# feifeibear/long-context-attention

Hardware: AMD Instinct MI355X
Metric: attention TFLOP/s (algorithmic, causal fwd+bwd) + iter ms of LongContextAttention at seqlen 64K, ulysses x ring (higher is better)
Workload: dtype bf16

## Files before the change

### include/usp_hip.h

```cpp
#ifndef USP_HIP_H
#define USP_HIP_H

#include <stdint.h>

#ifdef __cplusplus
extern "C" {
#endif

#define USP_ABI_VERSION 7

enum { USP_BF16 = 0, USP_FP16 = 1 };

enum {
  USP_OK = 0,
  USP_EINVAL = -1,
  USP_EUNSUPPORTED = -2,
  USP_ELAUNCH = -3
};

#define USP_LAUNCH_INTERLEAVE 1
#define USP_ATTN_WINDOW 2
#define USP_FORCE_ROW64 4
#define USP_FORCE_WAVE32 8
#define USP_BWD_SKIP_DQ 16
#define USP_BWD_SKIP_DKDV 32
#define USP_ATTN_SOFTCAP 64
#define USP_ATTN_SHIFT 128
#define USP_ATTN_ALIBI 256
#define USP_ATTN_DROPOUT 512
#define USP_ATTN_SINK 1024
#define USP_ATTN_DOC 2048
#define USP_ATTN_SPAN 4096
#define USP_ATTN_BLOCK_MASK 8192
#define USP_ATTN_MAX_LOGIT 16384
#define USP_ATTN_BLOCK_SELECT 32768

typedef struct usp_tensor {
  void* ptr;
  int64_t stride_b, stride_s, stride_h;
} usp_tensor;

typedef struct usp_fwd_args {
  int32_t dtype;
  int32_t B, Sq, Sk, Hq, Hkv, D;
  int32_t causal;
  float softmax_scale;
  int32_t mask_shift;
  usp_tensor q, k, v;
  usp_tensor out;
  usp_tensor acc;
  float* lse;
  int64_t lse_stride_b, lse_stride_h;
  int32_t merge_in;
  int32_t final_begin, final_end;
  const int32_t* seq_q;
  const int32_t* seq_k;
  int32_t* sched;
  int32_t flags;
  int32_t k_splits;
  void* workspace;
  int32_t window_left, window_right;
  float softcap;
} usp_fwd_args;

int usp_flash_fwd(const usp_fwd_args* args, void* stream);

int64_t usp_flash_fwd_workspace_bytes(const usp_fwd_args* args, int32_t k_splits);

typedef struct usp_bwd_args {
  int32_t dtype;
  int32_t B, Sq, Sk, Hq, Hkv, D;
  int32_t causal;
  float softmax_scale;
  int32_t mask_shift;
  usp_tensor dout, q, k, v;
  const float* lse;
  const float* delta;
  int64_t lse_stride_b, lse_stride_h;
  int64_t delta_stride_b, delta_stride_h;
  usp_tensor dq, dk, dv;
  int32_t accum_dq, accum_dk, accum_dv;
  usp_tensor dq16, dk16, dv16;
  void* workspace;
  int64_t workspace_bytes;
  const int32_t* seq_q;
  const int32_t* seq_k;
  int64_t total_k;
  int32_t* sched;
  int32_t flags;
  int32_t dq_splits;
  int32_t dkdv_splits;
  int32_t window_left, window_right;
  int32_t dkdv_heads;
  float softcap;
} usp_bwd_args;

int usp_flash_bwd(const usp_bwd_args* args, void* stream);

int usp_flash_fwd_alibi(const usp_fwd_args* args, const float* alibi_slopes, int64_t alibi_stride_b, void* stream);
int usp_flash_bwd_alibi(const usp_bwd_args* args, const float* alibi_slopes, int64_t alibi_stride_b, void* stream);

int usp_flash_fwd_dropout(const usp_fwd_args* args, float p_drop, uint64_t seed, int32_t row0, int32_t key0, int32_t head0,
                          void* stream);
int usp_flash_bwd_dropout(const usp_bwd_args* args, float p_drop, uint64_t seed, int32_t row0, int32_t key0, int32_t head0,
                          void* stream);

int usp_flash_fwd_sink(const usp_fwd_args* args, const float* sinks, void* stream);
int usp_sink_bwd(int32_t B, int32_t S, int32_t H, const float* sinks, const float* lse, int64_t lse_stride_b,
                 int64_t lse_stride_h, const float* delta, int64_t delta_stride_b, int64_t delta_stride_h, float* dsinks,
                 int32_t accum, void* stream);

int usp_flash_fwd_maxlogit(const usp_fwd_args* args, float* row_max, int64_t row_max_stride_b, int64_t row_max_stride_h,
                           void* stream);
int usp_row_max_reduce(int32_t B, int32_t S, int32_t H, const float* row_max, int64_t row_max_stride_b,
                       int64_t row_max_stride_h, float* out, int32_t accum, void* stream);

int usp_flash_fwd_doc(const usp_fwd_args* args, const int32_t* row_lo, int64_t row_lo_stride_b, void* stream);
int usp_flash_bwd_doc(const usp_bwd_args* args, const int32_t* row_lo, int64_t row_lo_stride_b, const int32_t* key_hi,
                      int64_t key_hi_stride_b, void* stream);

int usp_flash_fwd_span(const usp_fwd_args* args, const int32_t* row_lo, int64_t row_lo_stride_b, const int32_t* row_hi,
                       int64_t row_hi_stride_b, void* stream);
int usp_flash_bwd_span(const usp_bwd_args* args, const int32_t* row_lo, int64_t row_lo_stride_b, const int32_t* row_hi,
                       int64_t row_hi_stride_b, const int32_t* key_lo, int64_t key_lo_stride_b, const int32_t* key_hi,
                       int64_t key_hi_stride_b, void* stream);

#define USP_BLOCK_MASK_SIZE 128
int64_t usp_block_list_bytes(int32_t B, int32_t Hq, int32_t n_row_blocks, int32_t n_key_blocks);
int usp_block_lists_build(const void* mask, int64_t mask_stride_b, int64_t mask_stride_h, int64_t mask_stride_row, int32_t B, int32_t Hq,
                          int32_t S, int32_t causal, int32_t which, void* lists, void* stream);
int usp_flash_fwd_bsp(const usp_fwd_args* args, const void* mask, int64_t mask_stride_b, int64_t mask_stride_h,
                      int64_t mask_stride_row, void* lists, void* stream);
int usp_flash_bwd_bsp(const usp_bwd_args* args, const void* mask, int64_t mask_stride_b, int64_t mask_stride_h,
                      int64_t mask_stride_row, void* lists, void* stream);

#define USP_BLOCK_SELECT_MAX_BLOCKS 8192
int usp_block_means(const void* x, int32_t dtype, int32_t B, int32_t S, int32_t H, int32_t D, int64_t stride_b, int64_t stride_s,
                    int64_t stride_h, float* out, void* stream);
int usp_block_select(const float* qbar, const float* kbar, int32_t B, int32_t Hq, int32_t Hkv, int32_t D, int32_t nbq, int32_t nbk,
                     int32_t row_block0, float scale, int32_t causal, int32_t top_k, int32_t keep_first, int32_t keep_local,
                     void* mask, int64_t mask_stride_b, int64_t mask_stride_h, int64_t mask_stride_row, void* stream);

int64_t usp_flash_bwd_workspace_bytes(const usp_bwd_args* args);

int usp_bwd_delta(int32_t dtype, int32_t B, int32_t S, int32_t H, int32_t D,
                  const usp_tensor* dout, const usp_tensor* out,
                  float* delta, int64_t delta_stride_b, int64_t delta_stride_h, void* stream);

int usp_lse_merge(int32_t dtype, int32_t B, int32_t S, int32_t H, int32_t D,
                  const usp_tensor* acc, float* lse, int64_t lse_stride_b, int64_t lse_stride_h,
                  const usp_tensor* blk_out, const float* blk_lse, int64_t blk_lse_stride_b,
                  int64_t blk_lse_stride_h, int32_t first, void* stream);

int usp_copy_rows(void* dst, const void* src, int64_t row_bytes,
                  int64_t n0, int64_t n1, int64_t n2, int64_t n3,
                  int64_t ds0, int64_t ds1, int64_t ds2, int64_t ds3,
                  int64_t ss0, int64_t ss1, int64_t ss2, int64_t ss3, void* stream);

int usp_sum_rows(int32_t dtype, void* dst, const void* src, int64_t row_bytes, int32_t r, int64_t term_stride,
                 int64_t n0, int64_t n1, int64_t n2, int64_t ds0, int64_t ds1, int64_t ds2,
                 int64_t ss0, int64_t ss1, int64_t ss2, void* stream);

int usp_cast_from_f32(int32_t dtype, void* dst, int64_t dst_row_stride, const float* src,
                      int64_t src_row_stride, int64_t rows, int64_t n, void* stream);

int usp_add_f32(float* dst, int64_t dst_row_stride, const float* a, int64_t a_row_stride,
                const float* b, int64_t b_row_stride, int64_t rows, int64_t n, void* stream);

enum {
  USP_KIND_FWD_ROW64 = 1,
  USP_KIND_FWD_WAVE8 = 2,
  USP_KIND_FWD_WAVE4 = 4,
  USP_KIND_FWD_SPLIT_MERGE = 8,
  USP_KIND_DKDV_ROW64 = 16,
  USP_KIND_DKDV_WAVE8 = 32,
  USP_KIND_DQ_ROW64 = 64,
  USP_KIND_DQ_WAVE8 = 128,
  USP_KIND_REDUCE_HEADS = 256,
  USP_KIND_REDUCE_CUTS = 512
};
int usp_last_launch_kinds(void);

int usp_mfma_probe(const void* operands, int64_t operand_bytes, int32_t iters, int32_t waves_per_simd,
                   float* sink, uint64_t* clocks, void* stream);

int usp_abi_version(void);
int usp_attn_features(void);
const char* usp_strerror(int code);

#ifdef __cplusplus
}
#endif
#endif
```

### long-context-attention_amd/_C.py

```python
from __future__ import annotations

import ctypes
import math
import os
import struct
import threading
from typing import Optional

import torch

_HERE = os.path.dirname(os.path.abspath(__file__))
_LIB_PATH = os.path.join(_HERE, "libusp_hip.so")
_lib = None

USP_BF16, USP_FP16 = 0, 1
USP_LAUNCH_INTERLEAVE = 1
USP_ATTN_WINDOW = 2
USP_FORCE_ROW64 = 4
USP_FORCE_WAVE32 = 8
USP_BWD_SKIP_DQ = 16
USP_BWD_SKIP_DKDV = 32
USP_ATTN_SOFTCAP = 64
USP_ATTN_SHIFT = 128
USP_ATTN_ALIBI = 256
USP_ATTN_DROPOUT = 512
USP_ATTN_SINK = 1024
USP_ATTN_DOC = 2048
USP_ATTN_SPAN = 4096
USP_ATTN_BLOCK_MASK = 8192
USP_ATTN_MAX_LOGIT = 16384
USP_ATTN_BLOCK_SELECT = 32768
BLOCK_SELECT_MAX_BLOCKS = 8192
BLOCK_MASK_SIZE = 128
ABI_VERSION = 7
KINDS = {1: "fwd_row64", 2: "fwd_wave8", 4: "fwd_wave4", 8: "fwd_split_merge", 16: "dkdv_row64", 32: "dkdv_wave8",
         64: "dq_row64", 128: "dq_wave8", 256: "reduce_heads", 512: "reduce_cuts"}
_FAMILY_FLAG = {None: 0, "auto": 0, "row64": USP_FORCE_ROW64, "wave32": USP_FORCE_WAVE32}
_FAMILY_DEFAULT = "auto"


def set_kernel_family(family) -> str:
    global _FAMILY_DEFAULT
    if family not in _FAMILY_FLAG:
        raise ValueError(f"kernel family must be one of {sorted(k for k in _FAMILY_FLAG if k)}, got {family!r}")
    prev, _FAMILY_DEFAULT = _FAMILY_DEFAULT, (family or "auto")
    return prev


def _family_flag(family) -> int:
    if family is None:
        family = _FAMILY_DEFAULT
    try:
        return _FAMILY_FLAG[family]
    except KeyError:
        raise ValueError(f"kernel family must be one of {sorted(k for k in _FAMILY_FLAG if k)}, got {family!r}") from None


def last_launch_kinds() -> tuple:
    m = load().usp_last_launch_kinds()
    return tuple(name for bit, name in KINDS.items() if m & bit)


class UspTensor(ctypes.Structure):
    _fields_ = [("ptr", ctypes.c_void_p), ("stride_b", ctypes.c_int64),
                ("stride_s", ctypes.c_int64), ("stride_h", ctypes.c_int64)]


class UspFwdArgs(ctypes.Structure):
    _fields_ = [("dtype", ctypes.c_int32), ("B", ctypes.c_int32), ("Sq", ctypes.c_int32),
                ("Sk", ctypes.c_int32), ("Hq", ctypes.c_int32), ("Hkv", ctypes.c_int32),
                ("D", ctypes.c_int32), ("causal", ctypes.c_int32),
                ("softmax_scale", ctypes.c_float), ("mask_shift", ctypes.c_int32),
                ("q", UspTensor), ("k", UspTensor), ("v", UspTensor),
                ("out", UspTensor), ("acc", UspTensor),
                ("lse", ctypes.c_void_p), ("lse_stride_b", ctypes.c_int64),
                ("lse_stride_h", ctypes.c_int64),
                ("merge_in", ctypes.c_int32), ("final_begin", ctypes.c_int32),
                ("final_end", ctypes.c_int32),
                ("seq_q", ctypes.c_void_p), ("seq_k", ctypes.c_void_p), ("sched", ctypes.c_void_p),
                ("flags", ctypes.c_int32), ("k_splits", ctypes.c_int32), ("workspace", ctypes.c_void_p),
                ("window_left", ctypes.c_int32), ("window_right", ctypes.c_int32),
                ("softcap", ctypes.c_float)]


class UspBwdArgs(ctypes.Structure):
    _fields_ = [("dtype", ctypes.c_int32), ("B", ctypes.c_int32), ("Sq", ctypes.c_int32),
                ("Sk", ctypes.c_int32), ("Hq", ctypes.c_int32), ("Hkv", ctypes.c_int32),
                ("D", ctypes.c_int32), ("causal", ctypes.c_int32),
                ("softmax_scale", ctypes.c_float), ("mask_shift", ctypes.c_int32),
                ("dout", UspTensor), ("q", UspTensor), ("k", UspTensor), ("v", UspTensor),
                ("lse", ctypes.c_void_p), ("delta", ctypes.c_void_p),
                ("lse_stride_b", ctypes.c_int64), ("lse_stride_h", ctypes.c_int64),
                ("delta_stride_b", ctypes.c_int64), ("delta_stride_h", ctypes.c_int64),
                ("dq", UspTensor), ("dk", UspTensor), ("dv", UspTensor),
                ("accum_dq", ctypes.c_int32), ("accum_dk", ctypes.c_int32),
                ("accum_dv", ctypes.c_int32),
                ("dq16", UspTensor), ("dk16", UspTensor), ("dv16", UspTensor),
                ("workspace", ctypes.c_void_p), ("workspace_bytes", ctypes.c_int64),
                ("seq_q", ctypes.c_void_p), ("seq_k", ctypes.c_void_p), ("total_k", ctypes.c_int64),
                ("sched", ctypes.c_void_p), ("flags", ctypes.c_int32),
                ("dq_splits", ctypes.c_int32), ("dkdv_splits", ctypes.c_int32),
                ("window_left", ctypes.c_int32), ("window_right", ctypes.c_int32),
                ("dkdv_heads", ctypes.c_int32), ("softcap", ctypes.c_float)]


EXPORTS = ("usp_flash_fwd", "usp_flash_fwd_workspace_bytes", "usp_flash_bwd", "usp_flash_bwd_workspace_bytes", "usp_bwd_delta", "usp_lse_merge", "usp_copy_rows",
           "usp_sum_rows", "usp_cast_from_f32", "usp_add_f32", "usp_abi_version", "usp_strerror", "usp_last_launch_kinds", "usp_mfma_probe",
           "usp_attn_features", "usp_flash_fwd_alibi", "usp_flash_bwd_alibi", "usp_flash_fwd_dropout", "usp_flash_bwd_dropout",
           "usp_flash_fwd_sink", "usp_sink_bwd", "usp_flash_fwd_doc", "usp_flash_bwd_doc", "usp_flash_fwd_span", "usp_flash_bwd_span",
           "usp_block_list_bytes", "usp_block_lists_build", "usp_flash_fwd_bsp", "usp_flash_bwd_bsp",
           "usp_flash_fwd_maxlogit", "usp_row_max_reduce", "usp_block_means", "usp_block_select")
ALIBI_EXPORTS = ("usp_flash_fwd_alibi", "usp_flash_bwd_alibi")
DROPOUT_EXPORTS = ("usp_flash_fwd_dropout", "usp_flash_bwd_dropout")
SINK_EXPORTS = ("usp_flash_fwd_sink", "usp_sink_bwd")
DOC_EXPORTS = ("usp_flash_fwd_doc", "usp_flash_bwd_doc")
SPAN_EXPORTS = ("usp_flash_fwd_span", "usp_flash_bwd_span")
BSP_EXPORTS = ("usp_block_list_bytes", "usp_block_lists_build", "usp_flash_fwd_bsp", "usp_flash_bwd_bsp")
MAXL_EXPORTS = ("usp_flash_fwd_maxlogit", "usp_row_max_reduce")
SELECT_EXPORTS = ("usp_block_means", "usp_block_select")


def lib_path() -> str:
    return _LIB_PATH


def load():
    global _lib
    if _lib is not None:
        return _lib
    if not os.path.exists(_LIB_PATH):
        raise RuntimeError(
            f"libusp_hip.so not found at {_LIB_PATH}: the HIP extension is not built. Run "
            f"`python -c 'import __graft_entry__ as g; g.build()'` or "
            f"`make -C long-context-attention_amd/csrc`. There is no CPU fallback.")
    L = ctypes.CDLL(_LIB_PATH)
    for name in EXPORTS:
        if name not in ALIBI_EXPORTS + DROPOUT_EXPORTS + SINK_EXPORTS + DOC_EXPORTS + SPAN_EXPORTS + BSP_EXPORTS + MAXL_EXPORTS + SELECT_EXPORTS and not hasattr(L, name):
            raise RuntimeError(f"{_LIB_PATH} does not export {name} (stale build?)")
    L.usp_strerror.restype = ctypes.c_char_p
    L.usp_abi_version.restype = ctypes.c_int
    L.usp_last_launch_kinds.restype = ctypes.c_int
    L.usp_last_launch_kinds.argtypes = []
    L.usp_attn_features.restype = ctypes.c_int
    L.usp_attn_features.argtypes = []
    if L.usp_abi_version() != ABI_VERSION:
        raise RuntimeError(f"libusp_hip.so ABI {L.usp_abi_version()} != binding ABI {ABI_VERSION}")
    i32, i64, vp = ctypes.c_int32, ctypes.c_int64, ctypes.c_void_p
    L.usp_flash_fwd.argtypes = [ctypes.POINTER(UspFwdArgs), vp]
    L.usp_flash_bwd.argtypes = [ctypes.POINTER(UspBwdArgs), vp]
    L.usp_flash_fwd_workspace_bytes.argtypes = [ctypes.POINTER(UspFwdArgs), i32]
    L.usp_flash_fwd_workspace_bytes.restype = ctypes.c_int64
    L.usp_flash_bwd_workspace_bytes.argtypes = [ctypes.POINTER(UspBwdArgs)]
    L.usp_flash_bwd_workspace_bytes.restype = ctypes.c_int64
    L.usp_bwd_delta.argtypes = [i32, i32, i32, i32, i32, ctypes.POINTER(UspTensor),
                                ctypes.POINTER(UspTensor), vp, i64, i64, vp]
    L.usp_lse_merge.argtypes = [i32, i32, i32, i32, i32, ctypes.POINTER(UspTensor), vp, i64, i64,
                                ctypes.POINTER(UspTensor), vp, i64, i64, i32, vp]
    L.usp_copy_rows.argtypes = [vp, vp] + [i64] * 13 + [vp]
    L.usp_sum_rows.argtypes = [i32, vp, vp, i64, i32] + [i64] * 10 + [vp]
    L.usp_cast_from_f32.argtypes = [i32, vp, i64, vp, i64, i64, i64, vp]
    L.usp_add_f32.argtypes = [vp, i64, vp, i64, vp, i64, i64, i64, vp]
    L.usp_mfma_probe.argtypes = [vp, i64, i32, i32, vp, vp, vp]
    L.usp_mfma_probe.restype = ctypes.c_int
    for name in ("usp_flash_fwd", "usp_flash_bwd", "usp_bwd_delta", "usp_lse_merge", "usp_copy_rows", "usp_sum_rows",
                 "usp_cast_from_f32", "usp_add_f32"):
        getattr(L, name).restype = ctypes.c_int
    _lib = L
    return L


def _check(rc: int, what: str):
    if rc != 0:
        raise RuntimeError(f"{what} failed: {load().usp_strerror(rc).decode()} (code {rc})")


def _stream() -> ctypes.c_void_p:
    return ctypes.c_void_p(torch.cuda.current_stream().cuda_stream)


def dtype_code(dtype: torch.dtype) -> int:
    if dtype == torch.bfloat16:
        return USP_BF16
    if dtype == torch.float16:
        return USP_FP16
    raise TypeError(f"libusp_hip supports bfloat16 / float16 inputs, got {dtype}")


def _require_cuda(*tensors):
    for t in tensors:
        if t is not None and not t.is_cuda:
            raise RuntimeError(
                "libusp_hip kernels need ROCm device tensors (got a CPU tensor); there is no CPU "
                "fallback in this package")


def _t4(t: Optional[torch.Tensor]) -> UspTensor:
    if t is None:
        return UspTensor(None, 0, 0, 0)
    assert t.dim() == 4, t.shape
    if t.stride(3) != 1:
        raise ValueError("last (head_dim) stride must be 1")
    return UspTensor(t.data_ptr(), t.stride(0), t.stride(1), t.stride(2))


def _lse3(t: torch.Tensor):
    assert t.dim() == 3 and t.dtype == torch.float32
    if t.shape[2] > 1 and t.stride(2) != 1:
        raise ValueError("lse/delta must have unit stride along the sequence")
    return ctypes.c_void_p(t.data_ptr()), t.stride(0), t.stride(1)


_FWD_WS = {}


def _parse_ksplit(raw) -> object:
    raw = (raw or "auto").strip().lower()
    if raw in ("auto", "0"):
        return "auto" if raw == "auto" else 0
    try:
        n = int(raw)
    except ValueError:
        import warnings
        warnings.warn(f"USP_FWD_KSPLIT={raw!r} is neither 'auto', 0 nor an integer: the K split stays off")
        return 0
    return 0 if n < 2 else min(n, 8)


_KSPLIT_MODE = _parse_ksplit(os.environ.get("USP_FWD_KSPLIT"))


def set_fwd_ksplit(mode) -> object:
    global _KSPLIT_MODE
    prev, _KSPLIT_MODE = _KSPLIT_MODE, _parse_ksplit(str(mode))
    return prev


def fwd_k_splits(B: int, Sq: int, Hq: int, causal: bool) -> int:
    mode = _KSPLIT_MODE
    if mode == 0 or not causal:
        return 0
    items = B * Hq * ((Sq + 255) // 256)
    if items >= 512:
        return 0
    if mode == "auto":
        return 0 if Sq < 4096 else (2 if items >= 256 else 4)
    return mode


_BWD_SPLIT_MODE = _parse_ksplit(os.environ.get("USP_BWD_SPLIT"))


def set_bwd_split(mode) -> object:
    global _BWD_SPLIT_MODE
    prev, _BWD_SPLIT_MODE = _BWD_SPLIT_MODE, _parse_ksplit(str(mode))
    return prev


def bwd_splits(B: int, Sq: int, Sk: int, Hq: int, causal: bool):
    mode = _BWD_SPLIT_MODE
    if mode == 0:
        return 0, 0

    def cuts(items, rows):
        if rows < 4096 or items >= 512 or (items >= 256 and not causal):
            return 0
        if mode != "auto":
            return mode
        return 2 if items >= 256 else 4
    return cuts(B * Hq * ((Sq + 255) // 256), Sq), cuts(B * Hq * ((Sk + 127) // 128), Sk)


_TLS = threading.local()
_ARGS_CACHE_MAX = 64


def _strides(t):
    return None if t is None else t.stride()


def _window(window):
    if window is None:
        return None
    wl, wr = int(window[0]), int(window[1])
    return None if (wl < 0 and wr < 0) else (wl, wr)


def softcap_value(softcap) -> Optional[float]:
    if softcap is None:
        return None
    cap = float(softcap)
    if cap == 0.0:
        return None
    if not (math.isfinite(cap) and cap > 0.0):
        raise ValueError(f"softcap must be a finite number > 0 (0 / None = off), got {softcap!r}")
    return cap


def _set_softcap(a, cap: Optional[float]):
    if cap is None:
        return
    L = load()
    if not (hasattr(L, "usp_attn_features") and L.usp_attn_features() & USP_ATTN_SOFTCAP):
        raise NotImplementedError(f"{_LIB_PATH} does not serve softcap (USP_ATTN_SOFTCAP): rebuild it")
    a.flags |= USP_ATTN_SOFTCAP
    a.softcap = cap


def alibi_value(alibi_slopes, B: int, Hq: int, device):
    if alibi_slopes is None:
        return None
    if not isinstance(alibi_slopes, torch.Tensor):
        raise ValueError(f"alibi_slopes must be a torch.Tensor, got {type(alibi_slopes).__name__}")
    if alibi_slopes.dtype != torch.float32:
        raise ValueError(f"alibi_slopes must be float32, got {alibi_slopes.dtype}")
    if tuple(alibi_slopes.shape) not in ((Hq,), (B, Hq)):
        raise ValueError(f"alibi_slopes must have shape ({Hq},) or ({B}, {Hq}), got {tuple(alibi_slopes.shape)}")
    if alibi_slopes.device != torch.device(device):
        raise ValueError(f"alibi_slopes is on {alibi_slopes.device}, the operands on {device}")
    t = alibi_slopes.contiguous()
    return t, (Hq if t.dim() == 2 else 0)


def dropout_value(dropout_p) -> Optional[float]:
    if dropout_p is None:
        return None
    p = float(dropout_p)
    if p == 0.0:
        return None
    if not (0.0 < p < 1.0):
        raise ValueError(f"dropout_p must lie in [0, 1) (0 / None = off), got {dropout_p!r}")
    return p


def dropout_threshold(p: float) -> int:
    f32 = lambda x: struct.unpack("f", struct.pack("f", x))[0]
    return min(256, max(1, round(f32(f32(1.0 - f32(p)) * 256.0))))


def dropout_args(dropout):
    if dropout is None:
        return None
    p, seed, row0, key0, head0 = dropout
    p = dropout_value(p)
    if p is None or dropout_threshold(p) == 256:
        return None
    seed, row0, key0, head0 = int(seed), int(row0), int(key0), int(head0)
    if not 0 <= seed < 1 << 64:
        raise ValueError(f"dropout seed must fit 64 unsigned bits, got {seed}")
    if min(row0, key0, head0) < 0 or max(row0, key0, head0) >= 1 << 31:
        raise ValueError(f"dropout offsets (row0, key0, head0) must lie in [0, 2^31), got {(row0, key0, head0)}")
    return p, seed, row0, key0, head0


def sinks_value(sinks, Hq: int, device, dtype=None):
    if sinks is None:
        return None
    if not isinstance(sinks, torch.Tensor):
        raise ValueError(f"sinks must be a torch.Tensor, got {type(sinks).__name__}")
    if tuple(sinks.shape) != (Hq,):
        raise ValueError(f"sinks must have shape ({Hq},): one logit per query head, got {tuple(sinks.shape)}")
    ok = (torch.float32,) + ((torch.bfloat16, torch.float16) if dtype is None else (dtype,))
    if sinks.dtype not in ok:
        raise ValueError(f"sinks must be float32 or the operands' 16-bit type, got {sinks.dtype}")
    if sinks.device != torch.device(device):
        raise ValueError(f"sinks is on {sinks.device}, the operands on {device}")
    return sinks.detach().float().contiguous()


def doc_value(doc, B: int, Sq: int, Sk: int, device):
    if doc is None:
        return None
    row_lo, key_hi = doc
    if row_lo is None and key_hi is None:
        return None

    def one(t, n, what):
        if t is None:
            return None, 0
        if not isinstance(t, torch.Tensor) or t.dtype != torch.int32:
            raise ValueError(f"doc {what} must be an int32 torch.Tensor")
        if tuple(t.shape) not in ((n,), (B, n)) or not t.is_contiguous():
            raise ValueError(f"doc {what} must be contiguous with shape ({n},) or ({B}, {n}), got {tuple(t.shape)}")
        if t.device != torch.device(device):
            raise ValueError(f"doc {what} is on {t.device}, the operands on {device}")
        return t, (n if t.dim() == 2 else 0)
    return one(row_lo, Sq, "row_lo"), one(key_hi, Sk, "key_hi")


def span_value(span, B: int, Sq: int, Sk: int, device):
    if span is None:
        return None
    if len(span) != 4:
        raise ValueError(f"span must be (row_lo, row_hi, key_lo, key_hi), got {len(span)} entries")
    if all(t is None for t in span):
        return None

    def one(t, n, what):
        if t is None:
            return None, 0
        if not isinstance(t, torch.Tensor) or t.dtype != torch.int32:
            raise ValueError(f"span {what} must be an int32 torch.Tensor")
        if tuple(t.shape) not in ((n,), (B, n)) or not t.is_contiguous():
            raise ValueError(f"span {what} must be contiguous with shape ({n},) or ({B}, {n}), got {tuple(t.shape)}")
        if t.device != torch.device(device):
            raise ValueError(f"span {what} is on {t.device}, the operands on {device}")
        return t, (n if t.dim() == 2 else 0)
    return tuple(one(t, n, what) for t, n, what in zip(span, (Sq, Sq, Sk, Sk), ("row_lo", "row_hi", "key_lo", "key_hi")))


def block_mask_value(mask, B: int, Hq: int, S: int, device):
    if mask is None:
        return None
    if not isinstance(mask, torch.Tensor) or mask.dtype != torch.bool:
        raise ValueError(f"block_mask must be a torch.bool tensor, got {getattr(mask, 'dtype', type(mask).__name__)}")
    nb = (S + BLOCK_MASK_SIZE - 1) // BLOCK_MASK_SIZE
    if tuple(mask.shape) not in ((nb, nb), (Hq, nb, nb), (B, Hq, nb, nb)):
        raise ValueError(f"block_mask must have shape ({nb}, {nb}), ({Hq}, {nb}, {nb}) or ({B}, {Hq}, {nb}, {nb}) "
                         f"({BLOCK_MASK_SIZE} x {BLOCK_MASK_SIZE} blocks of {S} rows), got {tuple(mask.shape)}")
    if mask.device != torch.device(device):
        raise ValueError(f"block_mask is on {mask.device}, the operands on {device}")
    m = mask.detach()
    if nb > 1 and m.stride(-1) != 1:
        m = m.contiguous()
    m = m.view(torch.uint8)
    sr = m.stride(-2) if nb > 1 else nb
    sh = m.stride(-3) if m.dim() >= 3 else 0
    sb = m.stride(0) if m.dim() == 4 else 0
    return m, sb, sh, sr


def block_list_bytes(B: int, Hq: int, nb: int) -> int:
    return int(_feature_entry("usp_block_list_bytes")(B, Hq, nb, nb))


def block_list_layout(B: int, Hq: int, nb: int) -> dict:
    nqb, lf = (nb + 1) // 2, 2 * nb + 2
    off_q = B * Hq * nb * lf
    return dict(fwd=(0, nb, lf), dq=(off_q, nqb, lf), dkdv=(off_q + B * Hq * nqb * lf, nb, lf), ints=off_q + B * Hq * (nqb + nb) * lf)


def block_lists_build(mask, B: int, Hq: int, S: int, causal: bool, lists, which: int = 7):
    m, sb, sh, sr = block_mask_value(mask, B, Hq, S, lists.device)
    _check(_feature_entry("usp_block_lists_build")(_ptr(m), sb, sh, sr, B, Hq, S, 1 if causal else 0, int(which), _ptr(lists), _stream()),
           "usp_block_lists_build")


def _bsp_call(which: str, a, bsp, lists=None):
    m, sb, sh, sr = bsp
    nb = (a.Sq + BLOCK_MASK_SIZE - 1) // BLOCK_MASK_SIZE
    need = block_list_bytes(a.B, a.Hq, nb)
    if lists is None:
        lists = torch.empty(need, dtype=torch.uint8, device=m.device)
    elif lists.numel() * lists.element_size() < need or not lists.is_contiguous() or lists.device != m.device:
        raise ValueError(f"bsp_lists must be a contiguous device tensor of at least {need} bytes")
    name = f"usp_flash_{which}_bsp"
    _check(_feature_entry(name)(ctypes.byref(a), _ptr(m), sb, sh, sr, _ptr(lists), _stream()), name)


def block_select_value(top_k, keep_first=0, keep_local=1, causal=False):
    for name, x in (("top_k", top_k), ("keep_first", keep_first), ("keep_local", keep_local)):
        if isinstance(x, bool) or not isinstance(x, int):
            raise ValueError(f"block_select: {name} must be an int, got {x!r}")
        if x < 0:
            raise ValueError(f"block_select: {name} must be >= 0, got {x}")
    if causal and keep_local < 1:
        raise ValueError(f"block_select: a causal selection needs keep_local >= 1 (every row keeps its own block), got {keep_local}")
    i32max = (1 << 31) - 1
    return min(top_k, i32max), min(keep_first, i32max), min(keep_local, i32max)


def block_means(x, out=None):
    _require_cuda(x)
    B, S, H, D = x.shape
    nb = (S + BLOCK_MASK_SIZE - 1) // BLOCK_MASK_SIZE
    if out is None:
        out = torch.empty((B, nb, H, D), dtype=torch.float32, device=x.device)
    elif out.dtype != torch.float32 or tuple(out.shape) != (B, nb, H, D) or not out.is_contiguous() or out.device != x.device:
        raise ValueError(f"block_means: out must be a contiguous fp32 ({B}, {nb}, {H}, {D}) tensor on {x.device}")
    t = _t4(x)
    _check(_feature_entry("usp_block_means")(t.ptr, dtype_code(x.dtype), B, S, H, D, t.stride_b, t.stride_s, t.stride_h, _ptr(out),
                                             _stream()), "usp_block_means")
    return out


def block_select(qbar, kbar, top_k, scale: float, causal: bool, keep_first: int = 0, keep_local: int = 1, row_block0: int = 0,
                 out=None):
    _require_cuda(qbar, kbar)
    B, nbq, Hq, D = qbar.shape
    nbk, Hkv = kbar.shape[1], kbar.shape[2]
    for t, shape in ((qbar, (B, nbq, Hq, D)), (kbar, (B, nbk, Hkv, D))):
        if t.dtype != torch.float32 or tuple(t.shape) != shape or not t.is_contiguous():
            raise ValueError(f"block_select: the means must be contiguous fp32 {shape} tensors, got {tuple(t.shape)} {t.dtype}")
    if out is None:
        out = torch.empty((B, Hq, nbq, nbk), dtype=torch.bool, device=qbar.device)
    elif out.dtype not in (torch.bool, torch.uint8) or tuple(out.shape) != (B, Hq, nbq, nbk) or (nbk > 1 and out.stride(-1) != 1) \
            or out.device != qbar.device:
        raise ValueError(f"block_select: out must be a torch.bool ({B}, {Hq}, {nbq}, {nbk}) tensor with unit last stride on {qbar.device}")
    _check(_feature_entry("usp_block_select")(_ptr(qbar), _ptr(kbar), B, Hq, Hkv, D, nbq, nbk, int(row_block0), float(scale),
                                              1 if causal else 0, int(top_k), int(keep_first), int(keep_local), _ptr(out),
                                              out.stride(0), out.stride(1), out.stride(2), _stream()), "usp_block_select")
    return out


def _feature_entries():
    i32, i64, u64, f32, vp = ctypes.c_int32, ctypes.c_int64, ctypes.c_uint64, ctypes.c_float, ctypes.c_void_p
    fwd, bwd = ctypes.POINTER(UspFwdArgs), ctypes.POINTER(UspBwdArgs)
    return {"usp_flash_fwd_alibi": (USP_ATTN_ALIBI, "alibi_slopes (USP_ATTN_ALIBI)", [fwd, vp, i64, vp]),
            "usp_flash_bwd_alibi": (USP_ATTN_ALIBI, "alibi_slopes (USP_ATTN_ALIBI)", [bwd, vp, i64, vp]),
            "usp_flash_fwd_dropout": (USP_ATTN_DROPOUT, "dropout_p (USP_ATTN_DROPOUT)", [fwd, f32, u64, i32, i32, i32, vp]),
            "usp_flash_bwd_dropout": (USP_ATTN_DROPOUT, "dropout_p (USP_ATTN_DROPOUT)", [bwd, f32, u64, i32, i32, i32, vp]),
            "usp_flash_fwd_sink": (USP_ATTN_SINK, "sinks (USP_ATTN_SINK)", [fwd, vp, vp]),
            "usp_sink_bwd": (USP_ATTN_SINK, "sinks (USP_ATTN_SINK)", [i32, i32, i32, vp, vp, i64, i64, vp, i64, i64, vp, i32, vp]),
            "usp_flash_fwd_doc": (USP_ATTN_DOC, "cu_doclens (USP_ATTN_DOC)", [fwd, vp, i64, vp]),
            "usp_flash_bwd_doc": (USP_ATTN_DOC, "cu_doclens (USP_ATTN_DOC)", [bwd, vp, i64, vp, i64, vp]),
            "usp_flash_fwd_span": (USP_ATTN_SPAN, "bidirectional (USP_ATTN_SPAN)", [fwd, vp, i64, vp, i64, vp]),
            "usp_flash_bwd_span": (USP_ATTN_SPAN, "bidirectional (USP_ATTN_SPAN)", [bwd, vp, i64, vp, i64, vp, i64, vp, i64, vp]),
            "usp_block_list_bytes": (USP_ATTN_BLOCK_MASK, "block_mask (USP_ATTN_BLOCK_MASK)", [i32, i32, i32, i32]),
            "usp_block_lists_build": (USP_ATTN_BLOCK_MASK, "block_mask (USP_ATTN_BLOCK_MASK)",
                                      [vp, i64, i64, i64, i32, i32, i32, i32, i32, vp, vp]),
            "usp_flash_fwd_bsp": (USP_ATTN_BLOCK_MASK, "block_mask (USP_ATTN_BLOCK_MASK)", [fwd, vp, i64, i64, i64, vp, vp]),
            "usp_flash_bwd_bsp": (USP_ATTN_BLOCK_MASK, "block_mask (USP_ATTN_BLOCK_MASK)", [bwd, vp, i64, i64, i64, vp, vp]),
            "usp_flash_fwd_maxlogit": (USP_ATTN_MAX_LOGIT, "return_max_logits (USP_ATTN_MAX_LOGIT)", [fwd, vp, i64, i64, vp]),
            "usp_row_max_reduce": (USP_ATTN_MAX_LOGIT, "return_max_logits (USP_ATTN_MAX_LOGIT)", [i32, i32, i32, vp, i64, i64, vp, i32, vp]),
            "usp_block_means": (USP_ATTN_BLOCK_SELECT, "block_select (USP_ATTN_BLOCK_SELECT)", [vp, i32, i32, i32, i32, i32, i64, i64, i64, vp, vp]),
            "usp_block_select": (USP_ATTN_BLOCK_SELECT, "block_select (USP_ATTN_BLOCK_SELECT)",
                                 [vp, vp, i32, i32, i32, i32, i32, i32, i32, f32, i32, i32, i32, i32, vp, i64, i64, i64, vp])}


_FEATURE_ENTRIES = _feature_entries()


def _feature_entry(name: str):
    bit, option, argtypes = _FEATURE_ENTRIES[name]
    L = load()
    if not (hasattr(L, "usp_attn_features") and L.usp_attn_features() & bit and hasattr(L, name)):
        raise NotImplementedError(f"{_LIB_PATH} does not serve {option}: rebuild it")
    fn = getattr(L, name)
    if fn.argtypes is None:
        fn.argtypes = argtypes
        fn.restype = ctypes.c_int64 if name == "usp_block_list_bytes" else ctypes.c_int
    return fn


_alibi_entry = _dropout_entry = _sink_entry = _doc_entry = _span_entry = _bsp_entry = _maxl_entry = _select_entry = _feature_entry


def _ptr(t):
    return ctypes.c_void_p(None if t is None else t.data_ptr())


def _set_shift(a, shift: Optional[int]):
    if shift is None:
        return
    L = load()
    if not (hasattr(L, "usp_attn_features") and L.usp_attn_features() & USP_ATTN_SHIFT):
        raise RuntimeError(f"{_LIB_PATH} does not serve a mask shift (USP_ATTN_SHIFT): rebuild it")
    a.flags |= USP_ATTN_SHIFT
    a.mask_shift = int(shift)


def _shift(shift) -> Optional[int]:
    if shift is None:
        return None
    s = int(shift)
    if abs(s) >= 1 << 30:
        raise ValueError(f"shift must lie inside (-2^30, 2^30), got {shift!r}")
    return s


def _flash_call(which: str, a, al, dr, sk, dc, sp=None, mx=None):
    if mx is not None:
        _maxl_alone(alibi=al, dropout=dr, sinks=sk, doc=dc, span=sp)
        name = "usp_flash_fwd_maxlogit"
        _check(_feature_entry(name)(ctypes.byref(a), *mx, _stream()), name)
        return
    if sp is not None:
        from .kernels.features import Features
        from .kernels.features import SPAN_ON
        Features(alibi=al, dropout=dr, sinks=sk, doc=SPAN_ON).check()
        if dc is not None:
            raise ValueError("a launch takes doc= or span=, not both: the span arrays hold the document bound")
        (rl, rl_sb), (rh, rh_sb), (kl, kl_sb), (kh, kh_sb) = sp
        name = f"usp_flash_{which}_span"
        extra = (_ptr(rl), rl_sb, _ptr(rh), rh_sb) + (() if which == "fwd" else (_ptr(kl), kl_sb, _ptr(kh), kh_sb))
        _check(_feature_entry(name)(ctypes.byref(a), *extra, _stream()), name)
        return
    if al is None and dr is None and sk is None and dc is None:
        name, extra = "usp_flash_" + which, ()
        fn = getattr(load(), name)
    else:
        from .kernels.features import Features
        Features(alibi=al, dropout=dr, sinks=sk, doc=dc).check()
        if dc is not None:
            (rl, rl_sb), (kh, kh_sb) = dc
            name = f"usp_flash_{which}_doc"
            extra = (_ptr(rl), rl_sb) if which == "fwd" else (_ptr(rl), rl_sb, _ptr(kh), kh_sb)
        elif sk is not None:
            name, extra = "usp_flash_fwd_sink", (_ptr(sk),)
        elif dr is not None:
            name, extra = f"usp_flash_{which}_dropout", dr
        else:
            name, extra = f"usp_flash_{which}_alibi", (_ptr(al[0]), al[1])
        fn = _feature_entry(name)
    _check(fn(ctypes.byref(a), *extra, _stream()), name)


def _fwd_args(q, k, v, softmax_scale, causal, lse, out, acc, merge_in, final_begin, final_end, interleave, n, window=None,
              family_flag=0, softcap=None, shift=None):
    key = (q.dtype, q.shape, q.stride(), k.shape, k.stride(), v.stride(), lse.stride(), _strides(out), _strides(acc),
           softmax_scale, causal, merge_in, final_begin, final_end, interleave, n, window, family_flag, softcap, shift)
    cache = _TLS.__dict__.setdefault("fwd", {})
    a = cache.get(key)
    if a is None:
        B, Sq, Hq, D = q.shape
        a = UspFwdArgs()
        a.dtype = dtype_code(q.dtype)
        a.B, a.Sq, a.Sk, a.Hq, a.Hkv, a.D = B, Sq, k.shape[1], Hq, k.shape[2], D
        a.causal = 1 if causal else 0
        a.softmax_scale = float(softmax_scale)
        a.q, a.k, a.v, a.out, a.acc = _t4(q), _t4(k), _t4(v), _t4(out), _t4(acc)
        a.lse, a.lse_stride_b, a.lse_stride_h = _lse3(lse)
        a.merge_in = 1 if merge_in else 0
        a.final_begin = final_begin
        a.final_end = Sq if final_end is None else final_end
        a.flags = (USP_LAUNCH_INTERLEAVE if interleave else 0) | family_flag
        if window is not None:
            a.flags |= USP_ATTN_WINDOW
            a.window_left, a.window_right = window
        _set_softcap(a, softcap)
        _set_shift(a, shift)
        a.k_splits = n if n > 1 else 0
        if len(cache) >= _ARGS_CACHE_MAX:
            cache.clear()
        cache[key] = a
        return a
    a.q.ptr, a.k.ptr, a.v.ptr, a.lse = q.data_ptr(), k.data_ptr(), v.data_ptr(), lse.data_ptr()
    a.out.ptr = None if out is None else out.data_ptr()
    a.acc.ptr = None if acc is None else acc.data_ptr()
    return a


def flash_fwd(q, k, v, softmax_scale: float, causal: bool, lse, out=None, acc=None,
              merge_in: bool = False, final_begin: int = 0, final_end: Optional[int] = None,
              interleave: bool = False, k_splits: Optional[int] = None, window=None, family=None, softcap=None, shift=None,
              alibi=None, dropout=None, sinks=None, doc=None, span=None, bsp=None, bsp_lists=None, row_max=None):
    _require_cuda(q, k, v, lse, out, acc, row_max)
    B, Sq, Hq, D = q.shape
    mx = row_max_value(row_max, B, Hq, Sq, q.device)
    bm = block_mask_value(bsp, B, Hq, Sq, q.device)
    if mx is not None:
        _maxl_alone(softcap=softcap_value(softcap), bsp=bm)
    if bm is not None:
        _bsp_alone(window=_window(window), softcap=softcap_value(softcap), shift=_shift(shift), alibi=alibi, dropout=dropout_args(dropout),
                   sinks=sinks, doc=doc_value(doc, B, Sq, k.shape[1], q.device), span=span_value(span, B, Sq, k.shape[1], q.device))
        a = _fwd_args(q, k, v, softmax_scale, bool(causal), lse, out, acc, bool(merge_in), final_begin, final_end,
                      bool(interleave), 0, None, _family_flag(family), None, None)
        _bsp_call("fwd", a, bm, bsp_lists)
        return
    cap = softcap_value(softcap)
    ff = _family_flag(family)
    win, sh = _window(window), _shift(shift)
    dc = doc_value(doc, B, Sq, k.shape[1], q.device)
    sp = span_value(span, B, Sq, k.shape[1], q.device)
    if k_splits is None:
        n = 0 if (sh is not None or dc is not None or sp is not None or mx is not None) else fwd_k_splits(B, Sq, Hq, causal)
    else:
        n = int(k_splits)
    a = _fwd_args(q, k, v, softmax_scale, bool(causal), lse, out, acc, bool(merge_in), final_begin, final_end,
                  bool(interleave), n, win, ff, cap, sh)
    L = load()
    if n > 1:
        need = L.usp_flash_fwd_workspace_bytes(ctypes.byref(a), n)
        key = (q.device.index, torch.cuda.current_stream().cuda_stream)
        ws = _FWD_WS.get(key)
        if ws is None or ws.numel() < need:
            ws = _FWD_WS[key] = torch.empty(need, dtype=torch.uint8, device=q.device)
        a.workspace = ws.data_ptr()
    al = alibi_value(alibi, B, Hq, q.device)
    dr = dropout_args(dropout)
    sk = sinks_value(sinks, Hq, q.device, q.dtype)
    _flash_call("fwd", a, al, dr, sk, dc, sp, mx)


def _maxl_alone(**others):
    for name, value in others.items():
        if value is not None:
            raise NotImplementedError(f"row_max together with {name} is not supported by the HIP attention kernels")


def row_max_value(row_max, B: int, Hq: int, Sq: int, device):
    if row_max is None:
        return None
    if not isinstance(row_max, torch.Tensor) or row_max.dtype != torch.float32:
        raise ValueError("row_max must be a float32 torch.Tensor")
    if tuple(row_max.shape) != (B, Hq, Sq):
        raise ValueError(f"row_max must have shape ({B}, {Hq}, {Sq}): one value per (batch, query head, row), got {tuple(row_max.shape)}")
    if row_max.device != torch.device(device):
        raise ValueError(f"row_max is on {row_max.device}, the operands on {device}")
    return _lse3(row_max)


def row_max_reduce(row_max, out=None, accum: bool = False):
    _require_cuda(row_max, out)
    B, H, S = row_max.shape
    mx = row_max_value(row_max, B, H, S, row_max.device)
    if out is None:
        if accum:
            raise ValueError("row_max_reduce: accum needs the buffer to take the maximum with")
        out = torch.empty(H, dtype=torch.float32, device=row_max.device)
    if out.dtype != torch.float32 or tuple(out.shape) != (H,) or not out.is_contiguous():
        raise ValueError("row_max_reduce: out must be a contiguous float32 (H,) tensor")
    _check(_feature_entry("usp_row_max_reduce")(B, S, H, *mx, _ptr(out), 1 if accum else 0, _stream()), "usp_row_max_reduce")
    return out


def _bsp_alone(**others):
    for name, value in others.items():
        if value is not None:
            raise NotImplementedError(f"bsp together with {name} is not supported by the HIP attention kernels")


def _t3(t: Optional[torch.Tensor]) -> UspTensor:
    if t is None:
        return UspTensor(None, 0, 0, 0)
    assert t.dim() == 3, t.shape
    if t.stride(2) != 1:
        raise ValueError("last (head_dim) stride must be 1")
    return UspTensor(t.data_ptr(), 0, t.stride(0), t.stride(1))


def _lse2(t: torch.Tensor):
    assert t.dim() == 2 and t.dtype == torch.float32
    if t.shape[1] > 1 and t.stride(1) != 1:
        raise ValueError("lse/delta must have unit stride along the tokens")
    return ctypes.c_void_p(t.data_ptr()), 0, t.stride(0)


def _seq(t: torch.Tensor, n: int) -> ctypes.c_void_p:
    if t.dtype != torch.int32 or tuple(t.shape) != (n, 2) or not t.is_contiguous():
        raise ValueError("sequence table must be a contiguous (num_seq, 2) int32 tensor")
    _require_cuda(t)
    return ctypes.c_void_p(t.data_ptr())


_SCHED = {}


def sched_block(device) -> torch.Tensor:
    key = (device.index, torch.cuda.current_stream(device).cuda_stream)
    blk = _SCHED.get(key)
    if blk is None:
        blk = _SCHED[key] = torch.zeros(16, dtype=torch.int32, device=device)
    return blk


def flash_fwd_packed(q, k, v, seq_q, seq_k, max_q: int, max_k: int, softmax_scale: float,
                     causal: bool, lse, out=None, acc=None, merge_in: bool = False,
                     final_begin: int = 0, final_end: int = 2, interleave: bool = False, softcap=None, sched: bool = True):
    _require_cuda(q, k, v, lse, out, acc)
    cap = softcap_value(softcap)
    n = seq_q.shape[0]
    a = UspFwdArgs()
    a.dtype = dtype_code(q.dtype)
    a.B, a.Sq, a.Sk, a.Hq, a.Hkv, a.D = n, int(max_q), int(max_k), q.shape[1], k.shape[1], q.shape[2]
    a.causal = 1 if causal else 0
    a.softmax_scale = float(softmax_scale)
    a.q, a.k, a.v, a.out, a.acc = _t3(q), _t3(k), _t3(v), _t3(out), _t3(acc)
    a.lse, a.lse_stride_b, a.lse_stride_h = _lse2(lse)
    a.merge_in = 1 if merge_in else 0
    a.final_begin, a.final_end = int(final_begin), int(final_end)
    a.seq_q, a.seq_k = _seq(seq_q, n), _seq(seq_k, n)
    a.sched = sched_block(q.device).data_ptr() if sched else None
    a.flags = USP_LAUNCH_INTERLEAVE if interleave else 0
    _set_softcap(a, cap)
    _check(load().usp_flash_fwd(ctypes.byref(a), _stream()), "usp_flash_fwd")


def flash_bwd_packed(dout, q, k, v, lse, delta, seq_q, seq_k, max_q: int, max_k: int, dq, dk, dv,
                     softmax_scale: float, causal: bool, accum_dq=False, accum_dk=False,
                     accum_dv=False, dq16=None, dk16=None, dv16=None, interleave: bool = False, softcap=None,
                     sched: bool = True):
    _require_cuda(dout, q, k, v, lse, delta, dq, dk, dv, dq16, dk16, dv16)
    cap = softcap_value(softcap)
    n = seq_q.shape[0]
    a = UspBwdArgs()
    a.dtype = dtype_code(q.dtype)
    a.B, a.Sq, a.Sk, a.Hq, a.Hkv, a.D = n, int(max_q), int(max_k), q.shape[1], k.shape[1], q.shape[2]
    a.causal = 1 if causal else 0
    a.softmax_scale = float(softmax_scale)
    a.dout, a.q, a.k, a.v = _t3(dout), _t3(q), _t3(k), _t3(v)
    a.lse, a.lse_stride_b, a.lse_stride_h = _lse2(lse)
    a.delta, a.delta_stride_b, a.delta_stride_h = _lse2(delta)
    for t in (dq, dk, dv):
        if t is not None and t.dtype != torch.float32:
            raise TypeError("dq/dk/dv buffers of usp_flash_bwd are fp32")
    a.dq, a.dk, a.dv = _t3(dq), _t3(dk), _t3(dv)
    a.dq16, a.dk16, a.dv16 = _t3(dq16), _t3(dk16), _t3(dv16)
    a.accum_dq, a.accum_dk, a.accum_dv = int(bool(accum_dq)), int(bool(accum_dk)), int(bool(accum_dv))
    a.seq_q, a.seq_k = _seq(seq_q, n), _seq(seq_k, n)
    a.sched = sched_block(q.device).data_ptr() if sched else None
    a.flags = USP_LAUNCH_INTERLEAVE if interleave else 0
    _set_softcap(a, cap)
    a.total_k = k.shape[0]
    L = load()
    need = L.usp_flash_bwd_workspace_bytes(ctypes.byref(a))
    ws = None
    if need > 0:
        ws = torch.empty(need, dtype=torch.uint8, device=q.device)
        a.workspace, a.workspace_bytes = ws.data_ptr(), need
    _check(L.usp_flash_bwd(ctypes.byref(a), _stream()), "usp_flash_bwd")


def bwd_delta(dout, out, delta):
    _require_cuda(dout, out, delta)
    B, S, H, D = dout.shape
    td, to = _t4(dout), _t4(out)
    p, sb, sh = _lse3(delta)
    _check(load().usp_bwd_delta(dtype_code(dout.dtype), B, S, H, D, ctypes.byref(td),
                                ctypes.byref(to), p, sb, sh, _stream()), "usp_bwd_delta")


def sink_grad(sinks, lse, delta, out=None, accum: bool = False):
    _require_cuda(sinks, lse, delta, out)
    B, H, S = lse.shape
    assert delta.shape == lse.shape, (delta.shape, lse.shape)
    sk = sinks_value(sinks, H, lse.device)
    if out is None:
        if accum:
            raise ValueError("sink_grad: accum needs the buffer to add to")
        out = torch.empty(H, dtype=torch.float32, device=lse.device)
    if out.dtype != torch.float32 or tuple(out.shape) != (H,) or not out.is_contiguous():
        raise ValueError("sink_grad: out must be a contiguous float32 (H,) tensor")
    pl, lsb, lsh = _lse3(lse)
    pd, dsb, dsh = _lse3(delta)
    _check(_feature_entry("usp_sink_bwd")(B, S, H, ctypes.c_void_p(sk.data_ptr()), pl, lsb, lsh, pd, dsb, dsh,
                                       ctypes.c_void_p(out.data_ptr()), 1 if accum else 0, _stream()), "usp_sink_bwd")
    return out


def flash_bwd(dout, q, k, v, lse, delta, dq, dk, dv, softmax_scale: float, causal: bool,
              accum_dq=False, accum_dk=False, accum_dv=False, dq16=None, dk16=None, dv16=None,
              interleave: bool = False, splits=None, window=None, family=None, only=None, dkdv_heads: int = 0,
              softcap=None, shift=None, alibi=None, dropout=None, doc=None, span=None, bsp=None, bsp_lists=None):
    _require_cuda(dout, q, k, v, lse, delta, dq, dk, dv, dq16, dk16, dv16)
    cap = softcap_value(softcap)
    B, Sq, Hq, D = q.shape
    Sk, Hkv = k.shape[1], k.shape[2]
    a = UspBwdArgs()
    a.dtype = dtype_code(q.dtype)
    a.B, a.Sq, a.Sk, a.Hq, a.Hkv, a.D = B, Sq, Sk, Hq, Hkv, D
    a.causal = 1 if causal else 0
    a.softmax_scale = float(softmax_scale)
    a.dout, a.q, a.k, a.v = _t4(dout), _t4(q), _t4(k), _t4(v)
    a.lse, a.lse_stride_b, a.lse_stride_h = _lse3(lse)
    a.delta, a.delta_stride_b, a.delta_stride_h = _lse3(delta)
    for t in (dq, dk, dv):
        if t is not None and t.dtype != torch.float32:
            raise TypeError("dq/dk/dv buffers of usp_flash_bwd are fp32")
    a.dq, a.dk, a.dv = _t4(dq), _t4(dk), _t4(dv)
    a.dq16, a.dk16, a.dv16 = _t4(dq16), _t4(dk16), _t4(dv16)
    a.accum_dq, a.accum_dk, a.accum_dv = int(bool(accum_dq)), int(bool(accum_dk)), int(bool(accum_dv))
    ff = _family_flag(family)
    a.flags = (USP_LAUNCH_INTERLEAVE if interleave else 0) | ff | {None: 0, "dkdv": USP_BWD_SKIP_DQ, "dq": USP_BWD_SKIP_DKDV}[only]
    sh = _shift(shift)
    dc = doc_value(doc, B, Sq, Sk, q.device)
    sp = span_value(span, B, Sq, Sk, q.device)
    bm = block_mask_value(bsp, B, Hq, Sq, q.device)
    if bm is not None:
        _bsp_alone(window=_window(window), softcap=cap, shift=sh, alibi=alibi, dropout=dropout_args(dropout), doc=dc, span=sp)
    if splits is None:
        a.dq_splits, a.dkdv_splits = (0, 0) if (sh is not None or dc is not None or sp is not None or bm is not None) else bwd_splits(B, Sq, Sk, Hq, bool(causal))
    else:
        a.dq_splits, a.dkdv_splits = splits
    a.dkdv_heads = int(dkdv_heads)
    win = _window(window)
    if win is not None:
        a.flags |= USP_ATTN_WINDOW
        a.window_left, a.window_right = win
    _set_softcap(a, cap)
    _set_shift(a, sh)
    L = load()
    need = L.usp_flash_bwd_workspace_bytes(ctypes.byref(a))
    ws = None
    if need > 0:
        ws = torch.empty(need, dtype=torch.uint8, device=q.device)
        a.workspace, a.workspace_bytes = ws.data_ptr(), need
    if bm is not None:
        _bsp_call("bwd", a, bm, bsp_lists)
        return
    al = alibi_value(alibi, B, Hq, q.device)
    dr = dropout_args(dropout)
    _flash_call("bwd", a, al, dr, None, dc, sp)


def lse_merge(acc, lse, blk_out, blk_lse, first: bool):
    _require_cuda(acc, lse, blk_out, blk_lse)
    B, S, H, D = acc.shape
    ta, tb = _t4(acc), _t4(blk_out)
    p, sb, sh = _lse3(lse)
    p2, sb2, sh2 = _lse3(blk_lse)
    _check(load().usp_lse_merge(dtype_code(blk_out.dtype), B, S, H, D, ctypes.byref(ta), p, sb, sh,
                                ctypes.byref(tb), p2, sb2, sh2, 1 if first else 0, _stream()),
           "usp_lse_merge")


def copy_rows(dst, src, row_bytes, sizes, dst_strides, src_strides):
    _require_cuda(dst, src)
    n = list(sizes) + [1] * (4 - len(sizes))
    ds = list(dst_strides) + [0] * (4 - len(dst_strides))
    ss = list(src_strides) + [0] * (4 - len(src_strides))
    _check(load().usp_copy_rows(ctypes.c_void_p(dst.data_ptr()), ctypes.c_void_p(src.data_ptr()),
                                row_bytes, *n, *ds, *ss, _stream()), "usp_copy_rows")


def sum_rows(dst, src, row_bytes, r, term_stride, sizes, dst_strides, src_strides):
    _require_cuda(dst, src)
    if dst.dtype != src.dtype:
        raise TypeError(f"usp_sum_rows: dst {dst.dtype} and src {src.dtype} differ")
    if len(sizes) > 3 or len(dst_strides) != len(sizes) or len(src_strides) != len(sizes):
        raise ValueError(f"usp_sum_rows takes up to 3 outer dims with one stride each: {sizes} {dst_strides} {src_strides}")
    n = list(sizes) + [1] * (3 - len(sizes))
    ds = list(dst_strides) + [0] * (3 - len(dst_strides))
    ss = list(src_strides) + [0] * (3 - len(src_strides))
    _check(load().usp_sum_rows(dtype_code(dst.dtype), ctypes.c_void_p(dst.data_ptr()), ctypes.c_void_p(src.data_ptr()),
                               int(row_bytes), int(r), int(term_stride), *n, *ds, *ss, _stream()), "usp_sum_rows")


def _rows2d(t: torch.Tensor):
    if t.is_contiguous():
        return 1, t.numel(), t.numel()
    if t.dim() == 4 and t[0].is_contiguous():
        return t.shape[0], t[0].numel(), t.stride(0)
    raise ValueError("expected a contiguous tensor or a batch of contiguous slices")


def cast_from_f32(dst16, src32):
    _require_cuda(dst16, src32)
    r1, n1, s1 = _rows2d(dst16)
    r2, n2, s2 = _rows2d(src32)
    if (r1, n1) != (r2, n2):
        r1, n1, s1, s2 = dst16.shape[0], dst16[0].numel(), dst16.stride(0), src32.stride(0)
        assert dst16[0].is_contiguous() and src32[0].is_contiguous()
    _check(load().usp_cast_from_f32(dtype_code(dst16.dtype), ctypes.c_void_p(dst16.data_ptr()), s1,
                                    ctypes.c_void_p(src32.data_ptr()), s2, r1, n1, _stream()),
           "usp_cast_from_f32")


def add_f32(dst, a, b):
    _require_cuda(dst, a, b)
    assert dst.shape == a.shape == b.shape
    if dst.is_contiguous() and a.is_contiguous() and b.is_contiguous():
        rows, n, sd, sa, sb_ = 1, dst.numel(), dst.numel(), a.numel(), b.numel()
    else:
        assert dst[0].is_contiguous() and a[0].is_contiguous() and b[0].is_contiguous()
        rows, n = dst.shape[0], dst[0].numel()
        sd, sa, sb_ = dst.stride(0), a.stride(0), b.stride(0)
    _check(load().usp_add_f32(ctypes.c_void_p(dst.data_ptr()), sd, ctypes.c_void_p(a.data_ptr()), sa,
                              ctypes.c_void_p(b.data_ptr()), sb_, rows, n, _stream()), "usp_add_f32")


def mfma_probe(operands: torch.Tensor, iters: int, waves_per_simd: int = 1, clocks: Optional[torch.Tensor] = None):
    _require_cuda(operands, clocks)
    assert operands.dtype == torch.bfloat16 and operands.is_contiguous() and operands.numel() >= 32768
    key = ("probe_sink", operands.device.index)
    sink = _SCHED.get(key)
    if sink is None:
        sink = _SCHED[key] = torch.zeros(512, dtype=torch.float32, device=operands.device)
    _check(load().usp_mfma_probe(ctypes.c_void_p(operands.data_ptr()), operands.numel() * 2, int(iters), int(waves_per_simd),
                                 ctypes.c_void_p(sink.data_ptr()), ctypes.c_void_p(clocks.data_ptr() if clocks is not None else None),
                                 _stream()), "usp_mfma_probe")
    cus = torch.cuda.get_device_properties(operands.device).multi_processor_count
    return cus * 4 * waves_per_simd * iters * 64 * 32768.0
```

### long-context-attention_amd/csrc/usp_bwd_params.hpp

```cpp
#pragma once
#include "usp_common.hpp"
#include "usp_dropout_rng.h"

namespace usp {

struct BwdParams {
  const char* dout; const char* q; const char* k; const char* v;
  const float* lse; const float* delta;
  float* dq; float* dk; float* dv;
  int64_t do_sb, do_ss, do_sh;
  int64_t q_sb, q_ss, q_sh;
  int64_t k_sb, k_ss, k_sh;
  int64_t v_sb, v_ss, v_sh;
  int64_t lse_sb, lse_sh, dl_sb, dl_sh;
  int64_t dq_sb, dq_ss, dq_sh;
  int64_t dk_sb, dk_ss, dk_sh;
  int64_t dv_sb, dv_ss, dv_sh;
  int B, Sq, Sk, Hq, Hkv, G, nblk;
  int n_items;
  int causal_off;
  float scale, scale_log2;
  int accum_dq, accum_dk, accum_dv;
  char* dq16; char* dk16; char* dv16;
  int64_t dq16_sb, dq16_ss, dq16_sh, dk16_sb, dk16_ss, dk16_sh, dv16_sb, dv16_ss, dv16_sh;
  float* ws_dk; float* ws_dv;
  int64_t ws_rows;
  int split;
  int gsub, ngrp;
  int qsplit;
  int ksplit;
  int nslab;
  float* ws_dq;
  int win_on, win_lo;
  const int* seq_q; const int* seq_k;
  int* sched;
  int sched_lds;
  int interleave;
  int walk_g;
  int wide16;
};

struct BwdSoftcap {
  int cap_on;
  float cap_log2;
  float tanh_k2;
};
struct BwdArgsSC : BwdParams, BwdSoftcap {};
struct BwdAlibi {
  const float* al_slopes;
  int64_t al_sb;
  int al_diag;
};
struct BwdArgsAL : BwdParams, BwdAlibi {};
struct BwdArgsDR : BwdParams, Dropout {};
struct BwdDoc {
  const int* row_lo;
  const int* key_hi;
  int64_t row_lo_sb, key_hi_sb;
};
struct BwdArgsDOC : BwdParams, BwdDoc {};
struct BwdSpan {
  const int* row_hi;
  const int* key_lo;
  int64_t row_hi_sb, key_lo_sb;
};
struct BwdArgsSPAN : BwdParams, BwdDoc, BwdSpan {};
#define USP_BWD_NO_SPAN                                          \
  [[maybe_unused]] constexpr bool SPAN = false;                  \
  [[maybe_unused]] constexpr const int* span_row_hi = nullptr;   \
  [[maybe_unused]] constexpr const int* span_key_lo = nullptr;   \
  [[maybe_unused]] constexpr int64_t span_rh_sb = 0, span_kl_sb = 0; \
  USP_BWD_NO_BSP
struct BwdBsp {
  const int* bsp_lists;
  int bsp_stride;
};
struct BwdArgsBSP : BwdParams, BwdBsp {};
#define USP_BWD_NO_BSP                                           \
  [[maybe_unused]] constexpr bool BSP = false;                   \
  [[maybe_unused]] constexpr const int* bsp_lists = nullptr;     \
  [[maybe_unused]] constexpr int bsp_stride = 0;

USP_DEV bool bind_sequence(BwdParams& p, int b, int64_t* ws_row0) {
  if (p.seq_q == nullptr) { *ws_row0 = (int64_t)b * p.Sk; return true; }
  const int qf = p.seq_q[2 * b], ql = p.seq_q[2 * b + 1];
  const int kf = p.seq_k[2 * b], kl = p.seq_k[2 * b + 1];
  *ws_row0 = kf;
  if (ql <= 0 || kl <= 0) return false;
  p.dout += 2 * qf * p.do_ss; p.q += 2 * qf * p.q_ss;
  p.k += 2 * kf * p.k_ss; p.v += 2 * kf * p.v_ss;
  p.lse += qf; p.delta += qf;
  if (p.dq) p.dq += qf * p.dq_ss;
  if (p.dk) p.dk += kf * p.dk_ss;
  if (p.dv) p.dv += kf * p.dv_ss;
  if (p.dq16) p.dq16 += 2 * qf * p.dq16_ss;
  if (p.dk16) p.dk16 += 2 * kf * p.dk16_ss;
  if (p.dv16) p.dv16 += 2 * kf * p.dv16_ss;
  p.Sq = ql; p.Sk = kl; p.causal_off = kl - ql;
  return true;
}

constexpr int kTile = 64;


template <int D> USP_DEV int tile_swz(int row) {
  if (D == 128) return ((row & 3) << 2) | ((row >> 2) & 3);
  if (D == 64) return (((row >> 1) & 1) << 2) | ((row >> 2) & 3);
  return (row >> 2) & 3;
}

bool launch_dkdv64(const BwdParams& p, int dtype, bool causal, hipStream_t st, int* rc);
bool dkdv64_serves(const BwdParams& p);
bool launch_dq64(const BwdParams& p, int dtype, bool causal, hipStream_t st, int* rc);
bool dq64_serves(const BwdParams& p);
int launch_dkdv_alibi(const BwdArgsAL& p, int D, int dtype, bool causal, int grid, size_t lds, hipStream_t st);
int launch_dq_alibi(const BwdArgsAL& p, int D, int dtype, bool causal, int grid, size_t lds, hipStream_t st);
int launch_dkdv_dropout(const BwdArgsDR& p, int D, int dtype, bool causal, int grid, size_t lds, hipStream_t st);
int launch_dq_dropout(const BwdArgsDR& p, int D, int dtype, bool causal, int grid, size_t lds, hipStream_t st);
int launch_dkdv_doc(const BwdArgsDOC& p, int D, int dtype, bool causal, int grid, size_t lds, hipStream_t st);
int launch_dq_doc(const BwdArgsDOC& p, int D, int dtype, bool causal, int grid, size_t lds, hipStream_t st);
int launch_dkdv_span(const BwdArgsSPAN& p, int D, int dtype, int grid, size_t lds, hipStream_t st);
int launch_dq_span(const BwdArgsSPAN& p, int D, int dtype, int grid, size_t lds, hipStream_t st);
int launch_dkdv_bsp(const BwdArgsBSP& p, int D, int dtype, bool causal, int grid, size_t lds, hipStream_t st);
int launch_dq_bsp(const BwdArgsBSP& p, int D, int dtype, bool causal, int grid, size_t lds, hipStream_t st);

}
```

### long-context-attention_amd/csrc/usp_flash_bwd.hip

```cpp
#include "usp_bwd_params.hpp"
#include "usp_host.hpp"

namespace usp {

#define USP_BWD_NO_ALIBI                            \
  constexpr bool AL = false;                        \
  constexpr const float* al_slopes = nullptr;       \
  constexpr int64_t al_sb = 0;                      \
  constexpr int al_diag = 0;                        \
  constexpr bool DR = false;                        \
  constexpr Dropout dr{};                           \
  constexpr bool DOC = false;                       \
  [[maybe_unused]] constexpr const int* doc_row_lo = nullptr;   \
  [[maybe_unused]] constexpr const int* doc_key_hi = nullptr;   \
  [[maybe_unused]] constexpr int64_t doc_rl_sb = 0, doc_kh_sb = 0;   \
  USP_BWD_NO_SPAN

template <int D, int DT, bool CAUSAL>
__global__ __launch_bounds__(512, 2) void flash_bwd_kernel(
    const BwdParams p_in) {
  constexpr bool SC = false;
  constexpr float sc_cl2 = 0.f, sc_k2 = 0.f;
  USP_BWD_NO_ALIBI
#include "usp_flash_bwd_dq_body.inc"
}

template <int D, int DT, bool CAUSAL>
__global__ __launch_bounds__(512, 2) void flash_bwd_softcap_kernel(const BwdArgsSC p_in) {
  constexpr bool SC = true;
  const float sc_cl2 = p_in.cap_log2, sc_k2 = p_in.tanh_k2;
  USP_BWD_NO_ALIBI
#include "usp_flash_bwd_dq_body.inc"
}


template <int D, int DT, bool CAUSAL>
__global__ __launch_bounds__(512, 2) void flash_bwd_dkdv_kernel(const BwdParams p_in) {
  constexpr bool SC = false;
  constexpr float sc_cl2 = 0.f, sc_k2 = 0.f;
  USP_BWD_NO_ALIBI
#include "usp_flash_bwd_dkdv_body.inc"
}

template <int D, int DT, bool CAUSAL>
__global__ __launch_bounds__(512, 2) void flash_bwd_dkdv_softcap_kernel(const BwdArgsSC p_in) {
  constexpr bool SC = true;
  const float sc_cl2 = p_in.cap_log2, sc_k2 = p_in.tanh_k2;
  USP_BWD_NO_ALIBI
#include "usp_flash_bwd_dkdv_body.inc"
}

template <int D, int DT>
__global__ __launch_bounds__(256) void reduce_heads_kernel(const BwdParams p) {
  using E = Elem<DT>;
  constexpr int C4 = D / 4;
  const int S = p.Sk, H = p.Hkv;
  const int64_t total = (int64_t)p.B * S * H * C4;
  const int64_t gstride = p.ws_rows * H * D;
  for (int64_t i = (int64_t)blockIdx.x * 256 + threadIdx.x; i < total; i += (int64_t)gridDim.x * 256) {
    const int c4 = (int)(i % C4);
    const int64_t r = i / C4;
    const int h = (int)(r % H);
    const int64_t bs = r / H;
    const int sidx = (int)(bs % S);
    const int b = (int)(bs / S);
    int64_t row = sidx, wrow = bs, bb = b;
    if (p.seq_k != nullptr) {
      if (sidx >= p.seq_k[2 * b + 1] || p.seq_q[2 * b + 1] <= 0) continue;
      row = wrow = p.seq_k[2 * b] + sidx;
      bb = 0;
    }
    const int64_t e = 4 * c4;
    float* pk = p.dk ? p.dk + bb * p.dk_sb + row * p.dk_ss + h * p.dk_sh + e : nullptr;
    float* pv = p.dv ? p.dv + bb * p.dv_sb + row * p.dv_ss + h * p.dv_sh + e : nullptr;
    f32x4 ak = p.accum_dk ? *(const f32x4*)pk : f32x4{0.f, 0.f, 0.f, 0.f};
    f32x4 av = p.accum_dv ? *(const f32x4*)pv : f32x4{0.f, 0.f, 0.f, 0.f};
    const int64_t o = (wrow * H + h) * D + e;
    for (int g = 0; g < p.nslab; ++g) {
      ak += *(const f32x4*)(p.ws_dk + g * gstride + o);
      av += *(const f32x4*)(p.ws_dv + g * gstride + o);
    }
    if (p.dk16) {
      char* hk = p.dk16 + 2 * (bb * p.dk16_sb + row * p.dk16_ss + h * p.dk16_sh + e);
      *(u32x2*)hk = u32x2{E::pack2(ak[0], ak[1]), E::pack2(ak[2], ak[3])};
    } else {
      *(f32x4*)pk = ak;
    }
    if (p.dv16) {
      char* hv = p.dv16 + 2 * (bb * p.dv16_sb + row * p.dv16_ss + h * p.dv16_sh + e);
      *(u32x2*)hv = u32x2{E::pack2(av[0], av[1]), E::pack2(av[2], av[3])};
    } else {
      *(f32x4*)pv = av;
    }
  }
}

template <int D, int DT>
__global__ __launch_bounds__(256) void reduce_cuts_kernel(const BwdParams p) {
  using E = Elem<DT>;
  constexpr int C4 = D / 4;
  const int64_t total = (int64_t)p.B * p.Sq * p.Hq * C4;
  const int64_t cstride = (int64_t)p.B * p.Sq * p.Hq * D;
  for (int64_t i = (int64_t)blockIdx.x * 256 + threadIdx.x; i < total; i += (int64_t)gridDim.x * 256) {
    const int c4 = (int)(i % C4);
    int64_t r = i / C4;
    const int h = (int)(r % p.Hq); r /= p.Hq;
    const int sidx = (int)(r % p.Sq);
    const int b = (int)(r / p.Sq);
    const int64_t e = 4 * c4;
    float* pq = p.dq ? p.dq + b * p.dq_sb + (int64_t)sidx * p.dq_ss + h * p.dq_sh + e : nullptr;
    f32x4 a = p.accum_dq ? *(const f32x4*)pq : f32x4{0.f, 0.f, 0.f, 0.f};
    const int64_t o = (((int64_t)b * p.Sq + sidx) * p.Hq + h) * D + e;
    for (int c = 0; c < p.ksplit; ++c) a += *(const f32x4*)(p.ws_dq + c * cstride + o);
    if (p.dq16) {
      char* hq = p.dq16 + 2 * (b * p.dq16_sb + (int64_t)sidx * p.dq16_ss + h * p.dq16_sh + e);
      *(u32x2*)hq = u32x2{E::pack2(a[0], a[1]), E::pack2(a[2], a[3])};
    } else {
      *(f32x4*)pq = a;
    }
  }
}

static int reduce_grid(int64_t items) { return (int)((items + 255) / 256 > 2048 ? 2048 : (items + 255) / 256); }

struct BwdExtras {
  BwdAlibi al{};
  DropoutCall dc{};
  BwdDoc doc{};
  BwdSpan span{};
  BspCall bsp{};
  Dropout dr{};
  bool any() const { return al.al_slopes || dr.t || doc.row_lo || doc.key_hi || span.row_hi || span.key_lo || bsp.mask; }
};

template <int D, int DT>
static int launch_dkdv(BwdArgsSC& p, const BwdExtras& x, bool causal, hipStream_t st, bool row64) {
  p.nblk = (p.Sk + 127) / 128;
  p.n_items = p.B * p.Hkv * p.nblk * p.ngrp * p.qsplit;
  int rc = USP_ELAUNCH;
  if (row64 && launch_dkdv64(p, DT, causal, st, &rc)) {
    if (rc != USP_OK) return rc;
    launch_kinds_note(USP_KIND_DKDV_ROW64);
  } else {
    if ((int64_t)p.Sq * p.q_ss * 2 >= (1LL << 31) || (int64_t)p.Sq * p.do_ss * 2 >= (1LL << 31)) return USP_EUNSUPPORTED;
    const int grid = persistent_grid(p.n_items, device_cus(), p.interleave);
    constexpr size_t lds = 3 * (2 * kTile * D * 2 + 2 * kTile * 4) + 4 * 2 * 4096;
    p.sched_lds = (int)lds;
    const size_t lds_q = lds + (p.sched ? 16 : 0);
    const BwdParams pb = p;
    if (x.al.al_slopes) {
      BwdArgsAL pa;
      static_cast<BwdParams&>(pa) = pb;
      static_cast<BwdAlibi&>(pa) = x.al;
      if (int rc2 = launch_dkdv_alibi(pa, D, DT, causal, grid, lds_q, st)) return rc2;
    } else if (x.dr.t) {
      BwdArgsDR pd;
      static_cast<BwdParams&>(pd) = pb;
      static_cast<Dropout&>(pd) = x.dr;
      if (int rc2 = launch_dkdv_dropout(pd, D, DT, causal, grid, lds_q, st)) return rc2;
    } else if (x.bsp.mask) {
      const BlockLists& bl = x.bsp.layout;
      BwdArgsBSP pd;
      static_cast<BwdParams&>(pd) = pb;
      pd.bsp_lists = x.bsp.lists + bl.off_t; pd.bsp_stride = bl.lt;
      if (int rc2 = launch_dkdv_bsp(pd, D, DT, causal, grid, lds_q, st)) return rc2;
    } else if (x.span.key_lo) {
      BwdArgsSPAN pd;
      static_cast<BwdParams&>(pd) = pb;
      static_cast<BwdDoc&>(pd) = x.doc;
      static_cast<BwdSpan&>(pd) = x.span;
      if (int rc2 = launch_dkdv_span(pd, D, DT, grid, lds_q, st)) return rc2;
    } else if (x.doc.key_hi) {
      BwdArgsDOC pd;
      static_cast<BwdParams&>(pd) = pb;
      static_cast<BwdDoc&>(pd) = x.doc;
      if (int rc2 = launch_dkdv_doc(pd, D, DT, causal, grid, lds_q, st)) return rc2;
    } else
    with_causal(causal, [&](auto c) {
      constexpr bool C = decltype(c)::value;
      if (p.cap_on) hipLaunchKernelGGL((flash_bwd_dkdv_softcap_kernel<D, DT, C>), dim3(grid), dim3(512), lds_q, st, p);
      else hipLaunchKernelGGL((flash_bwd_dkdv_kernel<D, DT, C>), dim3(grid), dim3(512), lds_q, st, pb);
    });
    launch_kinds_note(USP_KIND_DKDV_WAVE8);
    if (launched() != USP_OK) return USP_ELAUNCH;
  }
  if (!p.split) return USP_OK;
  const BwdParams pb = p;
  hipLaunchKernelGGL((reduce_heads_kernel<D, DT>), dim3(reduce_grid((int64_t)p.B * p.Sk * p.Hkv * (D / 4))), dim3(256), 0, st, pb);
  if (launched() != USP_OK) return USP_ELAUNCH;
  launch_kinds_note(USP_KIND_REDUCE_HEADS);
  return USP_OK;
}

template <int D, int DT>
static int launch_dq(BwdArgsSC& p, const BwdExtras& x, bool causal, hipStream_t st, bool row64) {
  int rc = USP_ELAUNCH;
  if (row64 && launch_dq64(p, DT, causal, st, &rc)) {
    if (rc == USP_OK) launch_kinds_note(USP_KIND_DQ_ROW64);
    return rc;
  }
  p.nblk = (p.Sq + 255) / 256;
  p.n_items = p.B * p.Hq * p.nblk * p.ksplit;
  const int grid = persistent_grid(p.n_items, device_cus(), p.interleave);
  constexpr size_t lds = 2 * (2 * kTile * D * 2);
  p.sched_lds = (int)lds;
  const size_t lds_q = lds + (p.sched ? 16 : 0);
  const BwdParams pb = p;
  if (x.al.al_slopes) {
    BwdArgsAL pa;
    static_cast<BwdParams&>(pa) = pb;
    static_cast<BwdAlibi&>(pa) = x.al;
    if (int rc2 = launch_dq_alibi(pa, D, DT, causal, grid, lds_q, st)) return rc2;
  } else if (x.dr.t) {
    BwdArgsDR pd;
    static_cast<BwdParams&>(pd) = pb;
    static_cast<Dropout&>(pd) = x.dr;
    if (int rc2 = launch_dq_dropout(pd, D, DT, causal, grid, lds_q, st)) return rc2;
  } else if (x.bsp.mask) {
    const BlockLists& bl = x.bsp.layout;
    BwdArgsBSP pd;
    static_cast<BwdParams&>(pd) = pb;
    pd.bsp_lists = x.bsp.lists + bl.off_q; pd.bsp_stride = bl.lf;
    if (int rc2 = launch_dq_bsp(pd, D, DT, causal, grid, lds_q, st)) return rc2;
  } else if (x.span.row_hi) {
    BwdArgsSPAN pd;
    static_cast<BwdParams&>(pd) = pb;
    static_cast<BwdDoc&>(pd) = x.doc;
    static_cast<BwdSpan&>(pd) = x.span;
    if (int rc2 = launch_dq_span(pd, D, DT, grid, lds_q, st)) return rc2;
  } else if (x.doc.row_lo) {
    BwdArgsDOC pd;
    static_cast<BwdParams&>(pd) = pb;
    static_cast<BwdDoc&>(pd) = x.doc;
    if (int rc2 = launch_dq_doc(pd, D, DT, causal, grid, lds_q, st)) return rc2;
  } else
  with_causal(causal, [&](auto c) {
    constexpr bool C = decltype(c)::value;
    if (p.cap_on) hipLaunchKernelGGL((flash_bwd_softcap_kernel<D, DT, C>), dim3(grid), dim3(512), lds_q, st, p);
    else hipLaunchKernelGGL((flash_bwd_kernel<D, DT, C>), dim3(grid), dim3(512), lds_q, st, pb);
  });
  if (launched() != USP_OK) return USP_ELAUNCH;
  launch_kinds_note(USP_KIND_DQ_WAVE8);
  return USP_OK;
}

template <int D, int DT>
static int launch_reduce_cuts(const BwdParams& p, hipStream_t st) {
  hipLaunchKernelGGL((reduce_cuts_kernel<D, DT>), dim3(reduce_grid((int64_t)p.B * p.Sq * p.Hq * (D / 4))), dim3(256), 0, st, p);
  launch_kinds_note(USP_KIND_REDUCE_CUTS);
  return launched();
}

template <int D, int DT>
static int launch_bwd(BwdArgsSC p, const BwdExtras& x, bool causal, hipStream_t st, int force, int skip) {
  const bool want_dkdv = !(skip & USP_BWD_SKIP_DKDV), want_dq = !(skip & USP_BWD_SKIP_DQ);
  if ((force & USP_FORCE_ROW64) && !(D == 128 && (!want_dkdv || dkdv64_serves(p)) && (!want_dq || dq64_serves(p))))
    return USP_EUNSUPPORTED;
  const bool row64 = D == 128 && !(force & USP_FORCE_WAVE32) && !p.cap_on && !x.any();
  int rc = USP_OK;
  if (x.bsp.mask) {
    rc = launch_block_lists(x.bsp.mask, x.bsp.sb, x.bsp.sh, x.bsp.sr, x.bsp.lists, x.bsp.layout, p.Sq, p.Sk, causal, (want_dq ? 2 : 0) | (want_dkdv ? 4 : 0), st);
    if (rc != USP_OK) return rc;
  }
  if (want_dkdv && (rc = launch_dkdv<D, DT>(p, x, causal, st, row64)) != USP_OK) return rc;
  if (want_dq && (rc = launch_dq<D, DT>(p, x, causal, st, row64)) == USP_OK && p.ksplit > 1) rc = launch_reduce_cuts<D, DT>(p, st);
  return rc;
}

}

static int cuts_of(int32_t n, bool packed) { return (packed || n < 2) ? 1 : (n > 8 ? 8 : n); }

static int dkdv_heads_of(const usp_bwd_args* a) {
  const int G = a->Hq / a->Hkv;
  if (a->dkdv_heads > 0) return (G % a->dkdv_heads == 0) ? a->dkdv_heads : -1;
  if (G <= 1) return 1;
  if (a->seq_q || a->seq_k) return 1;
  const int64_t base = (int64_t)a->B * a->Hkv * ((a->Sk + 127) / 128) * cuts_of(a->dkdv_splits, false);
  const bool triangles = usp::decode_mask(*a).causal;
  const int64_t want = (triangles ? 2LL : 1LL) * usp::device_cus();
  int best = 1;
  const int cap = triangles ? 2 : 4;
  for (int g = 2; g <= G && g <= cap; ++g)
    if (G % g == 0 && base * (G / g) >= want) best = g;
  return best;
}

struct BwdPlan {
  int gsub, ngrp;
  int qsplit, ksplit;
  int64_t ws_rows;
  int64_t dkdv_bytes, dq_bytes;
};
static BwdPlan plan_bwd(const usp_bwd_args* a) {
  const bool packed = a->seq_q || a->seq_k;
  BwdPlan pl;
  pl.gsub = dkdv_heads_of(a);
  pl.ngrp = pl.gsub < 1 ? 0 : (a->Hq / a->Hkv) / pl.gsub;
  pl.qsplit = cuts_of(a->dkdv_splits, packed);
  pl.ksplit = cuts_of(a->dq_splits, packed);
  pl.ws_rows = packed ? a->total_k : (int64_t)a->B * a->Sk;
  const int64_t slabs = (int64_t)pl.ngrp * pl.qsplit;
  pl.dkdv_bytes = slabs > 1 ? 2 * slabs * pl.ws_rows * a->Hkv * a->D * 4 : 0;
  pl.dq_bytes = pl.ksplit > 1 ? (int64_t)pl.ksplit * a->B * a->Sq * a->Hq * a->D * 4 : 0;
  return pl;
}

extern "C" int64_t usp_flash_bwd_workspace_bytes(const usp_bwd_args* a) {
  if (!a || a->Hkv <= 0 || a->Hq < a->Hkv || a->Hq % a->Hkv != 0) return 0;
  const BwdPlan pl = plan_bwd(a);
  return pl.dkdv_bytes + pl.dq_bytes;
}

static int flash_bwd_call(const usp_bwd_args* a_in, usp::BwdExtras x, void* stream) {
  const usp_bwd_args* a = a_in;
  using namespace usp;
  launch_kinds_reset();
  if (!a || !a->lse || !a->delta) return USP_EINVAL;
  if (int rc = check_force(a->flags)) return rc;
  const int skip = a->flags & (USP_BWD_SKIP_DQ | USP_BWD_SKIP_DKDV);
  if (skip == (USP_BWD_SKIP_DQ | USP_BWD_SKIP_DKDV)) return USP_EINVAL;
  if (int rc = check_problem(*a)) return rc;
  if (int rc = check_alibi(*a, x.al.al_slopes, x.al.al_sb)) return rc;
  if (int rc = check_dropout(*a, x.dc, &x.dr)) return rc;
  const BwdDoc& doc = x.doc;
  const bool has_doc = doc.row_lo || doc.key_hi;
  if (has_doc && ((!(skip & USP_BWD_SKIP_DQ) && !doc.row_lo) || (!(skip & USP_BWD_SKIP_DKDV) && !doc.key_hi))) return USP_EINVAL;
  const BwdSpan& span = x.span;
  const bool has_span = span.row_hi || span.key_lo;
  if (int rc = check_doc(*a, has_doc && !has_span, doc.row_lo_sb, doc.key_hi_sb)) return rc;
  if (has_span && ((!(skip & USP_BWD_SKIP_DQ) && !(doc.row_lo && span.row_hi)) || (!(skip & USP_BWD_SKIP_DKDV) && !(doc.key_hi && span.key_lo))))
    return USP_EINVAL;
  if (int rc = check_span(*a, has_span, doc.row_lo_sb, doc.key_hi_sb, span.row_hi_sb, span.key_lo_sb)) return rc;
  if (int rc = check_bsp(*a, x.bsp.mask, x.bsp.sb, x.bsp.sh, x.bsp.sr, x.bsp.lists)) return rc;
  const bool has_bsp = x.bsp.mask != nullptr;
  if (has_bsp) x.bsp.layout = block_lists(a->B, a->Hq, (a->Sq + 127) / 128, (a->Sk + 127) / 128);
  if (!a->dout.ptr || !a->q.ptr || !a->k.ptr || !a->v.ptr) return USP_EINVAL;
  const bool packed = a->seq_q != nullptr || a->seq_k != nullptr;
  if (packed && !(a->seq_q && a->seq_k && a->total_k > 0)) return USP_EINVAL;
  auto need32 = [](const usp_tensor& t32, const usp_tensor& t16, int accum) { return !t16.ptr || accum; };
  const bool want_dq = !(skip & USP_BWD_SKIP_DQ), want_dkdv = !(skip & USP_BWD_SKIP_DKDV);
  if ((want_dq && need32(a->dq, a->dq16, a->accum_dq) && !a->dq.ptr) || (want_dkdv && need32(a->dk, a->dk16, a->accum_dk) && !a->dk.ptr) ||
      (want_dkdv && need32(a->dv, a->dv16, a->accum_dv) && !a->dv.ptr))
    return USP_EINVAL;
  auto ok32 = [](const usp_tensor& t) { return !t.ptr || tensor_aligned(t, 16, 4); };
  auto ok16 = [](const usp_tensor& t) { return !t.ptr || tensor_aligned(t, 8, 4); };
  if (!tensor_aligned(a->dout, 16, 8) || !tensor_aligned(a->q, 16, 8) || !tensor_aligned(a->k, 16, 8) || !tensor_aligned(a->v, 16, 8) ||
      !ok32(a->dq) || !ok32(a->dk) || !ok32(a->dv) || !ok16(a->dq16) || !ok16(a->dk16) || !ok16(a->dv16))
    return USP_EUNSUPPORTED;
  const Mask mask = decode_mask(*a);
  if (packed && (mask.windowed || mask.shifted)) return USP_EUNSUPPORTED;
  if (a->dq_splits < 0 || a->dq_splits > 8 || a->dkdv_splits < 0 || a->dkdv_splits > 8) return USP_EINVAL;
  usp_bwd_args uncut;
  if (has_doc || has_span || has_bsp) { uncut = *a; uncut.dq_splits = 0; uncut.dkdv_splits = 0; a = &uncut; }
  const BwdPlan plan = plan_bwd(a);
  if (a->dkdv_heads < 0 || plan.gsub < 1) return USP_EINVAL;
  BwdArgsSC p;
  p.dout = (const char*)a->dout.ptr; p.q = (const char*)a->q.ptr;
  p.k = (const char*)a->k.ptr; p.v = (const char*)a->v.ptr;
  p.lse = a->lse; p.delta = a->delta;
  p.dq = (float*)a->dq.ptr; p.dk = (float*)a->dk.ptr; p.dv = (float*)a->dv.ptr;
  p.do_sb = a->dout.stride_b; p.do_ss = a->dout.stride_s; p.do_sh = a->dout.stride_h;
  p.q_sb = a->q.stride_b; p.q_ss = a->q.stride_s; p.q_sh = a->q.stride_h;
  p.k_sb = a->k.stride_b; p.k_ss = a->k.stride_s; p.k_sh = a->k.stride_h;
  p.v_sb = a->v.stride_b; p.v_ss = a->v.stride_s; p.v_sh = a->v.stride_h;
  p.lse_sb = a->lse_stride_b; p.lse_sh = a->lse_stride_h;
  p.dl_sb = a->delta_stride_b; p.dl_sh = a->delta_stride_h;
  p.dq_sb = a->dq.stride_b; p.dq_ss = a->dq.stride_s; p.dq_sh = a->dq.stride_h;
  p.dk_sb = a->dk.stride_b; p.dk_ss = a->dk.stride_s; p.dk_sh = a->dk.stride_h;
  p.dv_sb = a->dv.stride_b; p.dv_ss = a->dv.stride_s; p.dv_sh = a->dv.stride_h;
  p.B = a->B; p.Sq = a->Sq; p.Sk = a->Sk; p.Hq = a->Hq; p.Hkv = a->Hkv; p.G = a->Hq / a->Hkv;
  p.nblk = 0;
  mask.store(p);
  p.scale = a->softmax_scale;
  p.scale_log2 = a->softmax_scale * kLog2e;
  p.accum_dq = a->accum_dq ? 1 : 0; p.accum_dk = a->accum_dk ? 1 : 0; p.accum_dv = a->accum_dv ? 1 : 0;
  p.dq16 = (char*)a->dq16.ptr; p.dk16 = (char*)a->dk16.ptr; p.dv16 = (char*)a->dv16.ptr;
  p.dq16_sb = a->dq16.stride_b; p.dq16_ss = a->dq16.stride_s; p.dq16_sh = a->dq16.stride_h;
  p.dk16_sb = a->dk16.stride_b; p.dk16_ss = a->dk16.stride_s; p.dk16_sh = a->dk16.stride_h;
  p.dv16_sb = a->dv16.stride_b; p.dv16_ss = a->dv16.stride_s; p.dv16_sh = a->dv16.stride_h;
  p.seq_q = a->seq_q; p.seq_k = a->seq_k;
  p.sched = packed ? a->sched : nullptr;
  p.sched_lds = 0;
  p.interleave = (a->flags & USP_LAUNCH_INTERLEAVE) ? 1 : 0;
  p.walk_g = p.G;
  p.wide16 = 0;
  p.ws_rows = plan.ws_rows;
  if (packed) {
    p.do_sb = p.q_sb = p.k_sb = p.v_sb = p.lse_sb = p.dl_sb = 0;
    p.dq_sb = p.dk_sb = p.dv_sb = p.dq16_sb = p.dk16_sb = p.dv16_sb = 0;
  }
  p.split = 0; p.qsplit = 1; p.ksplit = 1; p.nslab = 1; p.ws_dk = nullptr; p.ws_dv = nullptr; p.ws_dq = nullptr;
  p.gsub = p.G; p.ngrp = 1;
  const int64_t need = plan.dkdv_bytes + plan.dq_bytes;
  if (need > 0 && a->workspace && a->workspace_bytes >= need && aligned(a->workspace, 16)) {
    if (plan.dkdv_bytes > 0) {
      p.split = 1;
      p.gsub = plan.gsub; p.ngrp = plan.ngrp; p.qsplit = plan.qsplit;
      p.nslab = p.ngrp * p.qsplit;
      p.ws_dk = (float*)a->workspace;
      p.ws_dv = p.ws_dk + plan.dkdv_bytes / 8;
    }
    p.ksplit = plan.ksplit;
    if (p.ksplit > 1) p.ws_dq = (float*)((char*)a->workspace + plan.dkdv_bytes);
  }
  x.al.al_diag = alibi_diag(*a);
  const int force = a->flags & (USP_FORCE_ROW64 | USP_FORCE_WAVE32);
  return with_head_dim_dtype(a->D, a->dtype, [&](auto d, auto dt) {
    return launch_bwd<decltype(d)::value, decltype(dt)::value>(p, x, mask.causal, (hipStream_t)stream, force, skip);
  });
}

extern "C" int usp_flash_bwd(const usp_bwd_args* a, void* stream) { return flash_bwd_call(a, usp::BwdExtras{}, stream); }

extern "C" int usp_flash_bwd_alibi(const usp_bwd_args* a, const float* alibi_slopes, int64_t alibi_stride_b, void* stream) {
  usp::BwdExtras x;
  x.al.al_slopes = alibi_slopes; x.al.al_sb = alibi_stride_b;
  return flash_bwd_call(a, x, stream);
}

extern "C" int usp_flash_bwd_dropout(const usp_bwd_args* a, float p_drop, uint64_t seed, int32_t row0, int32_t key0, int32_t head0,
                                     void* stream) {
  usp::BwdExtras x;
  x.dc = usp::DropoutCall{p_drop, seed, row0, key0, head0};
  return flash_bwd_call(a, x, stream);
}

extern "C" int usp_flash_bwd_doc(const usp_bwd_args* a, const int32_t* row_lo, int64_t row_lo_stride_b, const int32_t* key_hi,
                                 int64_t key_hi_stride_b, void* stream) {
  const bool any = row_lo || key_hi;
  usp::BwdExtras x;
  x.doc = usp::BwdDoc{row_lo, key_hi, any ? row_lo_stride_b : 0, any ? key_hi_stride_b : 0};
  return flash_bwd_call(a, x, stream);
}

extern "C" int usp_flash_bwd_span(const usp_bwd_args* a, const int32_t* row_lo, int64_t row_lo_stride_b, const int32_t* row_hi,
                                  int64_t row_hi_stride_b, const int32_t* key_lo, int64_t key_lo_stride_b, const int32_t* key_hi,
                                  int64_t key_hi_stride_b, void* stream) {
  const bool any = row_lo || key_hi, any_span = row_hi || key_lo;
  usp::BwdExtras x;
  x.doc = usp::BwdDoc{row_lo, key_hi, any ? row_lo_stride_b : 0, any ? key_hi_stride_b : 0};
  x.span = usp::BwdSpan{row_hi, key_lo, any_span ? row_hi_stride_b : 0, any_span ? key_lo_stride_b : 0};
  return flash_bwd_call(a, x, stream);
}

extern "C" int usp_flash_bwd_bsp(const usp_bwd_args* a, const void* mask, int64_t mask_stride_b, int64_t mask_stride_h,
                                 int64_t mask_stride_row, void* lists, void* stream) {
  usp::BwdExtras x;
  if (mask) x.bsp = usp::BspCall{mask, mask_stride_b, mask_stride_h, mask_stride_row, (int*)lists};
  return flash_bwd_call(a, x, stream);
}
```

Before: 1031.

## Add 256-key dK/dV backward kernel with software-pipelined MFMA schedule

Adds a new row64 dK/dV backward kernel in which each work item covers 256 keys instead of 128. It uses a hand-scheduled slot loop that interleaves MFMA chains, LDS reads, DMA pieces and exp/pack element work, with triple buffering. A heuristic picks the new kernel by default for D=128 unpacked, unwindowed, long-sequence problems that have enough work items, and new flags can force 128 or 256 keys. The goal is more reuse of Q/dO tiles per key block and better overlap of memory with matrix work. The cost is fewer work items, which can hurt load balance, plus heavy register pressure from the accumulator pinning.

```diff
diff --git a/include/usp_hip.h b/include/usp_hip.h
--- a/include/usp_hip.h
+++ b/include/usp_hip.h
@@ -34,6 +34,8 @@
 #define USP_ATTN_BLOCK_MASK 8192
 #define USP_ATTN_MAX_LOGIT 16384
 #define USP_ATTN_BLOCK_SELECT 32768
+#define USP_DKDV_KEYS256 65536
+#define USP_DKDV_KEYS128 131072
 
 typedef struct usp_tensor {
   void* ptr;
@@ -177,7 +179,8 @@
   USP_KIND_DQ_ROW64 = 64,
   USP_KIND_DQ_WAVE8 = 128,
   USP_KIND_REDUCE_HEADS = 256,
-  USP_KIND_REDUCE_CUTS = 512
+  USP_KIND_REDUCE_CUTS = 512,
+  USP_KIND_DKDV_KEYS256 = 1024
 };
 int usp_last_launch_kinds(void);
 
diff --git a/long-context-attention_amd/_C.py b/long-context-attention_amd/_C.py
--- a/long-context-attention_amd/_C.py
+++ b/long-context-attention_amd/_C.py
@@ -30,6 +30,8 @@
 USP_ATTN_BLOCK_MASK = 8192
 USP_ATTN_MAX_LOGIT = 16384
 USP_ATTN_BLOCK_SELECT = 32768
+USP_DKDV_KEYS256 = 65536
+USP_DKDV_KEYS128 = 131072
 BLOCK_SELECT_MAX_BLOCKS = 8192
 BLOCK_MASK_SIZE = 128
 ABI_VERSION = 7
@@ -54,6 +56,15 @@
         return _FAMILY_FLAG[family]
     except KeyError:
         raise ValueError(f"kernel family must be one of {sorted(k for k in _FAMILY_FLAG if k)}, got {family!r}") from None
+
+
+_DKDV_KEYS_FLAG = {0: 0, None: 0, 128: USP_DKDV_KEYS128, 256: USP_DKDV_KEYS256}
+USP_KIND_DKDV_KEYS256 = 1024
+
+
+def last_dkdv_item_keys() -> int:
+    m = load().usp_last_launch_kinds()
+    return 0 if not m & 16 else (256 if m & USP_KIND_DKDV_KEYS256 else 128)
 
 
 def last_launch_kinds() -> tuple:
@@ -841,7 +852,7 @@
 def flash_bwd(dout, q, k, v, lse, delta, dq, dk, dv, softmax_scale: float, causal: bool,
               accum_dq=False, accum_dk=False, accum_dv=False, dq16=None, dk16=None, dv16=None,
               interleave: bool = False, splits=None, window=None, family=None, only=None, dkdv_heads: int = 0,
-              softcap=None, shift=None, alibi=None, dropout=None, doc=None, span=None, bsp=None, bsp_lists=None):
+              softcap=None, shift=None, alibi=None, dropout=None, doc=None, span=None, bsp=None, bsp_lists=None, dkdv_keys: int = 0):
     _require_cuda(dout, q, k, v, lse, delta, dq, dk, dv, dq16, dk16, dv16)
     cap = softcap_value(softcap)
     B, Sq, Hq, D = q.shape
@@ -862,6 +873,9 @@
     a.accum_dq, a.accum_dk, a.accum_dv = int(bool(accum_dq)), int(bool(accum_dk)), int(bool(accum_dv))
     ff = _family_flag(family)
     a.flags = (USP_LAUNCH_INTERLEAVE if interleave else 0) | ff | {None: 0, "dkdv": USP_BWD_SKIP_DQ, "dq": USP_BWD_SKIP_DKDV}[only]
+    if dkdv_keys not in _DKDV_KEYS_FLAG:
+        raise ValueError(f"dkdv_keys must be 0, 128 or 256, got {dkdv_keys!r}")
+    a.flags |= _DKDV_KEYS_FLAG[dkdv_keys]
     sh = _shift(shift)
     dc = doc_value(doc, B, Sq, Sk, q.device)
     sp = span_value(span, B, Sq, Sk, q.device)
diff --git a/long-context-attention_amd/csrc/usp_bwd_params.hpp b/long-context-attention_amd/csrc/usp_bwd_params.hpp
--- a/long-context-attention_amd/csrc/usp_bwd_params.hpp
+++ b/long-context-attention_amd/csrc/usp_bwd_params.hpp
@@ -111,6 +111,8 @@
 
 bool launch_dkdv64(const BwdParams& p, int dtype, bool causal, hipStream_t st, int* rc);
 bool dkdv64_serves(const BwdParams& p);
+bool launch_dkdv64u(const BwdParams& p, int dtype, bool causal, hipStream_t st, int* rc);
+bool dkdv64u_serves(const BwdParams& p);
 bool launch_dq64(const BwdParams& p, int dtype, bool causal, hipStream_t st, int* rc);
 bool dq64_serves(const BwdParams& p);
 int launch_dkdv_alibi(const BwdArgsAL& p, int D, int dtype, bool causal, int grid, size_t lds, hipStream_t st);
diff --git a/long-context-attention_amd/csrc/usp_flash_bwd.hip b/long-context-attention_amd/csrc/usp_flash_bwd.hip
--- a/long-context-attention_amd/csrc/usp_flash_bwd.hip
+++ b/long-context-attention_amd/csrc/usp_flash_bwd.hip
@@ -134,11 +134,14 @@
 };
 
 template <int D, int DT>
-static int launch_dkdv(BwdArgsSC& p, const BwdExtras& x, bool causal, hipStream_t st, bool row64) {
+static int launch_dkdv(BwdArgsSC& p, const BwdExtras& x, bool causal, hipStream_t st, bool row64, int keys) {
   p.nblk = (p.Sk + 127) / 128;
   p.n_items = p.B * p.Hkv * p.nblk * p.ngrp * p.qsplit;
   int rc = USP_ELAUNCH;
-  if (row64 && launch_dkdv64(p, DT, causal, st, &rc)) {
+  if (row64 && keys == 256 && launch_dkdv64u(p, DT, causal, st, &rc)) {
+    if (rc != USP_OK) return rc;
+    launch_kinds_note(USP_KIND_DKDV_ROW64 | USP_KIND_DKDV_KEYS256);
+  } else if (row64 && launch_dkdv64(p, DT, causal, st, &rc)) {
     if (rc != USP_OK) return rc;
     launch_kinds_note(USP_KIND_DKDV_ROW64);
   } else {
@@ -252,17 +255,18 @@
 }
 
 template <int D, int DT>
-static int launch_bwd(BwdArgsSC p, const BwdExtras& x, bool causal, hipStream_t st, int force, int skip) {
+static int launch_bwd(BwdArgsSC p, const BwdExtras& x, bool causal, hipStream_t st, int force, int skip, int keys) {
   const bool want_dkdv = !(skip & USP_BWD_SKIP_DKDV), want_dq = !(skip & USP_BWD_SKIP_DQ);
   if ((force & USP_FORCE_ROW64) && !(D == 128 && (!want_dkdv || dkdv64_serves(p)) && (!want_dq || dq64_serves(p))))
     return USP_EUNSUPPORTED;
   const bool row64 = D == 128 && !(force & USP_FORCE_WAVE32) && !p.cap_on && !x.any();
+  if (want_dkdv && (force & (USP_DKDV_KEYS256 | USP_DKDV_KEYS128)) && !(row64 && dkdv64u_serves(p))) return USP_EUNSUPPORTED;
   int rc = USP_OK;
   if (x.bsp.mask) {
     rc = launch_block_lists(x.bsp.mask, x.bsp.sb, x.bsp.sh, x.bsp.sr, x.bsp.lists, x.bsp.layout, p.Sq, p.Sk, causal, (want_dq ? 2 : 0) | (want_dkdv ? 4 : 0), st);
     if (rc != USP_OK) return rc;
   }
-  if (want_dkdv && (rc = launch_dkdv<D, DT>(p, x, causal, st, row64)) != USP_OK) return rc;
+  if (want_dkdv && (rc = launch_dkdv<D, DT>(p, x, causal, st, row64, keys)) != USP_OK) return rc;
   if (want_dq && (rc = launch_dq<D, DT>(p, x, causal, st, row64)) == USP_OK && p.ksplit > 1) rc = launch_reduce_cuts<D, DT>(p, st);
   return rc;
 }
@@ -271,12 +275,20 @@
 
 static int cuts_of(int32_t n, bool packed) { return (packed || n < 2) ? 1 : (n > 8 ? 8 : n); }
 
-static int dkdv_heads_of(const usp_bwd_args* a) {
+static int dkdv_keys_of(const usp_bwd_args* a) {
+  if (a->flags & USP_DKDV_KEYS256) return 256;
+  if (a->flags & USP_DKDV_KEYS128) return 128;
+  if (a->D != 128 || a->seq_q || a->seq_k || (a->flags & (USP_FORCE_WAVE32 | USP_ATTN_SOFTCAP)) || usp::decode_mask(*a).windowed) return 128;
+  const int64_t items = (int64_t)a->B * a->Hq * ((a->Sk + 255) / 256);
+  return (a->Sq >= 8192 && items >= 4LL * usp::device_cus()) ? 256 : 128;
+}
+
+static int dkdv_heads_of(const usp_bwd_args* a, int keys) {
   const int G = a->Hq / a->Hkv;
   if (a->dkdv_heads > 0) return (G % a->dkdv_heads == 0) ? a->dkdv_heads : -1;
   if (G <= 1) return 1;
   if (a->seq_q || a->seq_k) return 1;
-  const int64_t base = (int64_t)a->B * a->Hkv * ((a->Sk + 127) / 128) * cuts_of(a->dkdv_splits, false);
+  const int64_t base = (int64_t)a->B * a->Hkv * ((a->Sk + keys - 1) / keys) * cuts_of(a->dkdv_splits, false);
   const bool triangles = usp::decode_mask(*a).causal;
   const int64_t want = (triangles ? 2LL : 1LL) * usp::device_cus();
   int best = 1;
@@ -287,6 +299,7 @@
 }
 
 struct BwdPlan {
+  int keys;
   int gsub, ngrp;
   int qsplit, ksplit;
   int64_t ws_rows;
@@ -295,7 +308,8 @@
 static BwdPlan plan_bwd(const usp_bwd_args* a) {
   const bool packed = a->seq_q || a->seq_k;
   BwdPlan pl;
-  pl.gsub = dkdv_heads_of(a);
+  pl.keys = dkdv_keys_of(a);
+  pl.gsub = dkdv_heads_of(a, pl.keys);
   pl.ngrp = pl.gsub < 1 ? 0 : (a->Hq / a->Hkv) / pl.gsub;
   pl.qsplit = cuts_of(a->dkdv_splits, packed);
   pl.ksplit = cuts_of(a->dq_splits, packed);
@@ -318,6 +332,8 @@
   launch_kinds_reset();
   if (!a || !a->lse || !a->delta) return USP_EINVAL;
   if (int rc = check_force(a->flags)) return rc;
+  if ((a->flags & USP_DKDV_KEYS256) && (a->flags & (USP_DKDV_KEYS128 | USP_FORCE_WAVE32))) return USP_EINVAL;
+  if ((a->flags & USP_DKDV_KEYS128) && (a->flags & USP_FORCE_WAVE32)) return USP_EINVAL;
   const int skip = a->flags & (USP_BWD_SKIP_DQ | USP_BWD_SKIP_DKDV);
   if (skip == (USP_BWD_SKIP_DQ | USP_BWD_SKIP_DKDV)) return USP_EINVAL;
   if (int rc = check_problem(*a)) return rc;
@@ -405,9 +421,9 @@
     if (p.ksplit > 1) p.ws_dq = (float*)((char*)a->workspace + plan.dkdv_bytes);
   }
   x.al.al_diag = alibi_diag(*a);
-  const int force = a->flags & (USP_FORCE_ROW64 | USP_FORCE_WAVE32);
+  const int force = a->flags & (USP_FORCE_ROW64 | USP_FORCE_WAVE32 | USP_DKDV_KEYS256 | USP_DKDV_KEYS128);
   return with_head_dim_dtype(a->D, a->dtype, [&](auto d, auto dt) {
-    return launch_bwd<decltype(d)::value, decltype(dt)::value>(p, x, mask.causal, (hipStream_t)stream, force, skip);
+    return launch_bwd<decltype(d)::value, decltype(dt)::value>(p, x, mask.causal, (hipStream_t)stream, force, skip, plan.keys);
   });
 }
 
diff --git a/long-context-attention_amd/csrc/usp_flash_bwd64u.hip b/long-context-attention_amd/csrc/usp_flash_bwd64u.hip
--- /dev/null
+++ b/long-context-attention_amd/csrc/usp_flash_bwd64u.hip
@@ -0,0 +1,471 @@
+#ifdef USP_B64U_TIMING
+#define USP_TIMING
+#endif
+#include "usp_bwd_params.hpp"
+#include "usp_host.hpp"
+#include "usp_mfma64.hpp"
+#include <utility>
+
+namespace usp {
+
+#ifndef USP_B64U_PE0
+#define USP_B64U_PE0 17
+#endif
+#ifndef USP_B64U_PE1
+#define USP_B64U_PE1 33
+#endif
+#ifndef USP_B64U_SE0
+#define USP_B64U_SE0 33
+#endif
+#ifndef USP_B64U_SE1
+#define USP_B64U_SE1 55
+#endif
+#ifndef USP_B64U_LA
+#define USP_B64U_LA 3
+#endif
+constexpr int kU_PE0 = USP_B64U_PE0, kU_PE1 = USP_B64U_PE1, kU_SE0 = USP_B64U_SE0, kU_SE1 = USP_B64U_SE1;
+constexpr int kU_LA = USP_B64U_LA;
+
+#define USP_U_ACC16(X) \
+  X(0, "a[0:15]", "v_accvgpr_read_b32 %0, a0\n\tv_accvgpr_read_b32 %1, a1\n\tv_accvgpr_read_b32 %2, a2\n\tv_accvgpr_read_b32 %3, a3\n\tv_accvgpr_read_b32 %4, a4\n\tv_accvgpr_read_b32 %5, a5\n\tv_accvgpr_read_b32 %6, a6\n\tv_accvgpr_read_b32 %7, a7\n\tv_accvgpr_read_b32 %8, a8\n\tv_accvgpr_read_b32 %9, a9\n\tv_accvgpr_read_b32 %10, a10\n\tv_accvgpr_read_b32 %11, a11\n\tv_accvgpr_read_b32 %12, a12\n\tv_accvgpr_read_b32 %13, a13\n\tv_accvgpr_read_b32 %14, a14\n\tv_accvgpr_read_b32 %15, a15", "a0", "a1", "a2", "a3", "a4", "a5", "a6", "a7", "a8", "a9", "a10", "a11", "a12", "a13", "a14", "a15") \
+  X(1, "a[16:31]", "v_accvgpr_read_b32 %0, a16\n\tv_accvgpr_read_b32 %1, a17\n\tv_accvgpr_read_b32 %2, a18\n\tv_accvgpr_read_b32 %3, a19\n\tv_accvgpr_read_b32 %4, a20\n\tv_accvgpr_read_b32 %5, a21\n\tv_accvgpr_read_b32 %6, a22\n\tv_accvgpr_read_b32 %7, a23\n\tv_accvgpr_read_b32 %8, a24\n\tv_accvgpr_read_b32 %9, a25\n\tv_accvgpr_read_b32 %10, a26\n\tv_accvgpr_read_b32 %11, a27\n\tv_accvgpr_read_b32 %12, a28\n\tv_accvgpr_read_b32 %13, a29\n\tv_accvgpr_read_b32 %14, a30\n\tv_accvgpr_read_b32 %15, a31", "a16", "a17", "a18", "a19", "a20", "a21", "a22", "a23", "a24", "a25", "a26", "a27", "a28", "a29", "a30", "a31") \
+  X(2, "a[32:47]", "v_accvgpr_read_b32 %0, a32\n\tv_accvgpr_read_b32 %1, a33\n\tv_accvgpr_read_b32 %2, a34\n\tv_accvgpr_read_b32 %3, a35\n\tv_accvgpr_read_b32 %4, a36\n\tv_accvgpr_read_b32 %5, a37\n\tv_accvgpr_read_b32 %6, a38\n\tv_accvgpr_read_b32 %7, a39\n\tv_accvgpr_read_b32 %8, a40\n\tv_accvgpr_read_b32 %9, a41\n\tv_accvgpr_read_b32 %10, a42\n\tv_accvgpr_read_b32 %11, a43\n\tv_accvgpr_read_b32 %12, a44\n\tv_accvgpr_read_b32 %13, a45\n\tv_accvgpr_read_b32 %14, a46\n\tv_accvgpr_read_b32 %15, a47", "a32", "a33", "a34", "a35", "a36", "a37", "a38", "a39", "a40", "a41", "a42", "a43", "a44", "a45", "a46", "a47") \
+  X(3, "a[48:63]", "v_accvgpr_read_b32 %0, a48\n\tv_accvgpr_read_b32 %1, a49\n\tv_accvgpr_read_b32 %2, a50\n\tv_accvgpr_read_b32 %3, a51\n\tv_accvgpr_read_b32 %4, a52\n\tv_accvgpr_read_b32 %5, a53\n\tv_accvgpr_read_b32 %6, a54\n\tv_accvgpr_read_b32 %7, a55\n\tv_accvgpr_read_b32 %8, a56\n\tv_accvgpr_read_b32 %9, a57\n\tv_accvgpr_read_b32 %10, a58\n\tv_accvgpr_read_b32 %11, a59\n\tv_accvgpr_read_b32 %12, a60\n\tv_accvgpr_read_b32 %13, a61\n\tv_accvgpr_read_b32 %14, a62\n\tv_accvgpr_read_b32 %15, a63", "a48", "a49", "a50", "a51", "a52", "a53", "a54", "a55", "a56", "a57", "a58", "a59", "a60", "a61", "a62", "a63") \
+  X(4, "a[64:79]", "v_accvgpr_read_b32 %0, a64\n\tv_accvgpr_read_b32 %1, a65\n\tv_accvgpr_read_b32 %2, a66\n\tv_accvgpr_read_b32 %3, a67\n\tv_accvgpr_read_b32 %4, a68\n\tv_accvgpr_read_b32 %5, a69\n\tv_accvgpr_read_b32 %6, a70\n\tv_accvgpr_read_b32 %7, a71\n\tv_accvgpr_read_b32 %8, a72\n\tv_accvgpr_read_b32 %9, a73\n\tv_accvgpr_read_b32 %10, a74\n\tv_accvgpr_read_b32 %11, a75\n\tv_accvgpr_read_b32 %12, a76\n\tv_accvgpr_read_b32 %13, a77\n\tv_accvgpr_read_b32 %14, a78\n\tv_accvgpr_read_b32 %15, a79", "a64", "a65", "a66", "a67", "a68", "a69", "a70", "a71", "a72", "a73", "a74", "a75", "a76", "a77", "a78", "a79") \
+  X(5, "a[80:95]", "v_accvgpr_read_b32 %0, a80\n\tv_accvgpr_read_b32 %1, a81\n\tv_accvgpr_read_b32 %2, a82\n\tv_accvgpr_read_b32 %3, a83\n\tv_accvgpr_read_b32 %4, a84\n\tv_accvgpr_read_b32 %5, a85\n\tv_accvgpr_read_b32 %6, a86\n\tv_accvgpr_read_b32 %7, a87\n\tv_accvgpr_read_b32 %8, a88\n\tv_accvgpr_read_b32 %9, a89\n\tv_accvgpr_read_b32 %10, a90\n\tv_accvgpr_read_b32 %11, a91\n\tv_accvgpr_read_b32 %12, a92\n\tv_accvgpr_read_b32 %13, a93\n\tv_accvgpr_read_b32 %14, a94\n\tv_accvgpr_read_b32 %15, a95", "a80", "a81", "a82", "a83", "a84", "a85", "a86", "a87", "a88", "a89", "a90", "a91", "a92", "a93", "a94", "a95") \
+  X(6, "a[96:111]", "v_accvgpr_read_b32 %0, a96\n\tv_accvgpr_read_b32 %1, a97\n\tv_accvgpr_read_b32 %2, a98\n\tv_accvgpr_read_b32 %3, a99\n\tv_accvgpr_read_b32 %4, a100\n\tv_accvgpr_read_b32 %5, a101\n\tv_accvgpr_read_b32 %6, a102\n\tv_accvgpr_read_b32 %7, a103\n\tv_accvgpr_read_b32 %8, a104\n\tv_accvgpr_read_b32 %9, a105\n\tv_accvgpr_read_b32 %10, a106\n\tv_accvgpr_read_b32 %11, a107\n\tv_accvgpr_read_b32 %12, a108\n\tv_accvgpr_read_b32 %13, a109\n\tv_accvgpr_read_b32 %14, a110\n\tv_accvgpr_read_b32 %15, a111", "a96", "a97", "a98", "a99", "a100", "a101", "a102", "a103", "a104", "a105", "a106", "a107", "a108", "a109", "a110", "a111") \
+  X(7, "a[112:127]", "v_accvgpr_read_b32 %0, a112\n\tv_accvgpr_read_b32 %1, a113\n\tv_accvgpr_read_b32 %2, a114\n\tv_accvgpr_read_b32 %3, a115\n\tv_accvgpr_read_b32 %4, a116\n\tv_accvgpr_read_b32 %5, a117\n\tv_accvgpr_read_b32 %6, a118\n\tv_accvgpr_read_b32 %7, a119\n\tv_accvgpr_read_b32 %8, a120\n\tv_accvgpr_read_b32 %9, a121\n\tv_accvgpr_read_b32 %10, a122\n\tv_accvgpr_read_b32 %11, a123\n\tv_accvgpr_read_b32 %12, a124\n\tv_accvgpr_read_b32 %13, a125\n\tv_accvgpr_read_b32 %14, a126\n\tv_accvgpr_read_b32 %15, a127", "a112", "a113", "a114", "a115", "a116", "a117", "a118", "a119", "a120", "a121", "a122", "a123", "a124", "a125", "a126", "a127") \
+  X(8, "a[128:143]", "v_accvgpr_read_b32 %0, a128\n\tv_accvgpr_read_b32 %1, a129\n\tv_accvgpr_read_b32 %2, a130\n\tv_accvgpr_read_b32 %3, a131\n\tv_accvgpr_read_b32 %4, a132\n\tv_accvgpr_read_b32 %5, a133\n\tv_accvgpr_read_b32 %6, a134\n\tv_accvgpr_read_b32 %7, a135\n\tv_accvgpr_read_b32 %8, a136\n\tv_accvgpr_read_b32 %9, a137\n\tv_accvgpr_read_b32 %10, a138\n\tv_accvgpr_read_b32 %11, a139\n\tv_accvgpr_read_b32 %12, a140\n\tv_accvgpr_read_b32 %13, a141\n\tv_accvgpr_read_b32 %14, a142\n\tv_accvgpr_read_b32 %15, a143", "a128", "a129", "a130", "a131", "a132", "a133", "a134", "a135", "a136", "a137", "a138", "a139", "a140", "a141", "a142", "a143") \
+  X(9, "a[144:159]", "v_accvgpr_read_b32 %0, a144\n\tv_accvgpr_read_b32 %1, a145\n\tv_accvgpr_read_b32 %2, a146\n\tv_accvgpr_read_b32 %3, a147\n\tv_accvgpr_read_b32 %4, a148\n\tv_accvgpr_read_b32 %5, a149\n\tv_accvgpr_read_b32 %6, a150\n\tv_accvgpr_read_b32 %7, a151\n\tv_accvgpr_read_b32 %8, a152\n\tv_accvgpr_read_b32 %9, a153\n\tv_accvgpr_read_b32 %10, a154\n\tv_accvgpr_read_b32 %11, a155\n\tv_accvgpr_read_b32 %12, a156\n\tv_accvgpr_read_b32 %13, a157\n\tv_accvgpr_read_b32 %14, a158\n\tv_accvgpr_read_b32 %15, a159", "a144", "a145", "a146", "a147", "a148", "a149", "a150", "a151", "a152", "a153", "a154", "a155", "a156", "a157", "a158", "a159") \
+  X(10, "a[160:175]", "v_accvgpr_read_b32 %0, a160\n\tv_accvgpr_read_b32 %1, a161\n\tv_accvgpr_read_b32 %2, a162\n\tv_accvgpr_read_b32 %3, a163\n\tv_accvgpr_read_b32 %4, a164\n\tv_accvgpr_read_b32 %5, a165\n\tv_accvgpr_read_b32 %6, a166\n\tv_accvgpr_read_b32 %7, a167\n\tv_accvgpr_read_b32 %8, a168\n\tv_accvgpr_read_b32 %9, a169\n\tv_accvgpr_read_b32 %10, a170\n\tv_accvgpr_read_b32 %11, a171\n\tv_accvgpr_read_b32 %12, a172\n\tv_accvgpr_read_b32 %13, a173\n\tv_accvgpr_read_b32 %14, a174\n\tv_accvgpr_read_b32 %15, a175", "a160", "a161", "a162", "a163", "a164", "a165", "a166", "a167", "a168", "a169", "a170", "a171", "a172", "a173", "a174", "a175") \
+  X(11, "a[176:191]", "v_accvgpr_read_b32 %0, a176\n\tv_accvgpr_read_b32 %1, a177\n\tv_accvgpr_read_b32 %2, a178\n\tv_accvgpr_read_b32 %3, a179\n\tv_accvgpr_read_b32 %4, a180\n\tv_accvgpr_read_b32 %5, a181\n\tv_accvgpr_read_b32 %6, a182\n\tv_accvgpr_read_b32 %7, a183\n\tv_accvgpr_read_b32 %8, a184\n\tv_accvgpr_read_b32 %9, a185\n\tv_accvgpr_read_b32 %10, a186\n\tv_accvgpr_read_b32 %11, a187\n\tv_accvgpr_read_b32 %12, a188\n\tv_accvgpr_read_b32 %13, a189\n\tv_accvgpr_read_b32 %14, a190\n\tv_accvgpr_read_b32 %15, a191", "a176", "a177", "a178", "a179", "a180", "a181", "a182", "a183", "a184", "a185", "a186", "a187", "a188", "a189", "a190", "a191") \
+  X(12, "a[192:207]", "v_accvgpr_read_b32 %0, a192\n\tv_accvgpr_read_b32 %1, a193\n\tv_accvgpr_read_b32 %2, a194\n\tv_accvgpr_read_b32 %3, a195\n\tv_accvgpr_read_b32 %4, a196\n\tv_accvgpr_read_b32 %5, a197\n\tv_accvgpr_read_b32 %6, a198\n\tv_accvgpr_read_b32 %7, a199\n\tv_accvgpr_read_b32 %8, a200\n\tv_accvgpr_read_b32 %9, a201\n\tv_accvgpr_read_b32 %10, a202\n\tv_accvgpr_read_b32 %11, a203\n\tv_accvgpr_read_b32 %12, a204\n\tv_accvgpr_read_b32 %13, a205\n\tv_accvgpr_read_b32 %14, a206\n\tv_accvgpr_read_b32 %15, a207", "a192", "a193", "a194", "a195", "a196", "a197", "a198", "a199", "a200", "a201", "a202", "a203", "a204", "a205", "a206", "a207") \
+  X(13, "a[208:223]", "v_accvgpr_read_b32 %0, a208\n\tv_accvgpr_read_b32 %1, a209\n\tv_accvgpr_read_b32 %2, a210\n\tv_accvgpr_read_b32 %3, a211\n\tv_accvgpr_read_b32 %4, a212\n\tv_accvgpr_read_b32 %5, a213\n\tv_accvgpr_read_b32 %6, a214\n\tv_accvgpr_read_b32 %7, a215\n\tv_accvgpr_read_b32 %8, a216\n\tv_accvgpr_read_b32 %9, a217\n\tv_accvgpr_read_b32 %10, a218\n\tv_accvgpr_read_b32 %11, a219\n\tv_accvgpr_read_b32 %12, a220\n\tv_accvgpr_read_b32 %13, a221\n\tv_accvgpr_read_b32 %14, a222\n\tv_accvgpr_read_b32 %15, a223", "a208", "a209", "a210", "a211", "a212", "a213", "a214", "a215", "a216", "a217", "a218", "a219", "a220", "a221", "a222", "a223") \
+  X(14, "a[224:239]", "v_accvgpr_read_b32 %0, a224\n\tv_accvgpr_read_b32 %1, a225\n\tv_accvgpr_read_b32 %2, a226\n\tv_accvgpr_read_b32 %3, a227\n\tv_accvgpr_read_b32 %4, a228\n\tv_accvgpr_read_b32 %5, a229\n\tv_accvgpr_read_b32 %6, a230\n\tv_accvgpr_read_b32 %7, a231\n\tv_accvgpr_read_b32 %8, a232\n\tv_accvgpr_read_b32 %9, a233\n\tv_accvgpr_read_b32 %10, a234\n\tv_accvgpr_read_b32 %11, a235\n\tv_accvgpr_read_b32 %12, a236\n\tv_accvgpr_read_b32 %13, a237\n\tv_accvgpr_read_b32 %14, a238\n\tv_accvgpr_read_b32 %15, a239", "a224", "a225", "a226", "a227", "a228", "a229", "a230", "a231", "a232", "a233", "a234", "a235", "a236", "a237", "a238", "a239") \
+  X(15, "a[240:255]", "v_accvgpr_read_b32 %0, a240\n\tv_accvgpr_read_b32 %1, a241\n\tv_accvgpr_read_b32 %2, a242\n\tv_accvgpr_read_b32 %3, a243\n\tv_accvgpr_read_b32 %4, a244\n\tv_accvgpr_read_b32 %5, a245\n\tv_accvgpr_read_b32 %6, a246\n\tv_accvgpr_read_b32 %7, a247\n\tv_accvgpr_read_b32 %8, a248\n\tv_accvgpr_read_b32 %9, a249\n\tv_accvgpr_read_b32 %10, a250\n\tv_accvgpr_read_b32 %11, a251\n\tv_accvgpr_read_b32 %12, a252\n\tv_accvgpr_read_b32 %13, a253\n\tv_accvgpr_read_b32 %14, a254\n\tv_accvgpr_read_b32 %15, a255", "a240", "a241", "a242", "a243", "a244", "a245", "a246", "a247", "a248", "a249", "a250", "a251", "a252", "a253", "a254", "a255")
+template <int DT> struct MU;
+#if defined(__HIP_DEVICE_COMPILE__)
+#define USP_MU_ACC(i, tup, rd, ...) case i: asm volatile(USP_MU_MN " " tup ", %0, %1, " tup : : "v"(a), "v"(b) : __VA_ARGS__); break;
+#define USP_MU_ZERO(i, tup, rd, ...) case i: asm volatile(USP_MU_MN " " tup ", %0, %0, 0" : : "v"(z) : __VA_ARGS__); break;
+#define USP_MU_BODY                                                                                                    \
+   \
+  template <bool SAFE = false> static USP_DEV void chain(f32x16& s, const u32x4& a, const u32x4& b) {                   \
+    if (SAFE) asm volatile("s_nop 1\n\t" USP_MU_MN " %0, %1, %2, %0" : "+v"(s) : "v"(a), "v"(b));                     \
+    else asm volatile(USP_MU_MN " %0, %1, %2, %0" : "+v"(s) : "v"(a), "v"(b));                                          \
+  }                                                                                                                     \
+                             \
+  template <bool SAFE = false> static USP_DEV void grad(int ac, const u32x4& a, const u32x4& b) {                       \
+    if (SAFE) asm volatile("s_nop 1");                                                                                  \
+    switch (ac) { USP_U_ACC16(USP_MU_ACC) }                                                                             \
+  }                                                                                                                     \
+                   \
+  static USP_DEV void zero(int ac, const u32x4& z) {                                                                    \
+    asm volatile("s_nop 1");                                                                                            \
+    switch (ac) { USP_U_ACC16(USP_MU_ZERO) }                                                                            \
+  }
+#else
+#define USP_MU_BODY                                                                                                    \
+  template <bool SAFE = false> static USP_DEV void chain(f32x16&, const u32x4&, const u32x4&) {}                        \
+  template <bool SAFE = false> static USP_DEV void grad(int, const u32x4&, const u32x4&) {}                             \
+  static USP_DEV void zero(int, const u32x4&) {}
+#endif
+#define USP_MU_MN "v_mfma_f32_32x32x16_bf16"
+template <> struct MU<0> { USP_MU_BODY };
+#undef USP_MU_MN
+#define USP_MU_MN "v_mfma_f32_32x32x16_f16"
+template <> struct MU<1> { USP_MU_BODY };
+#undef USP_MU_MN
+
+USP_DEV void acc_read(int ac, f32x16& o) {
+#if defined(__HIP_DEVICE_COMPILE__)
+  float t[16];
+#define USP_MU_READ(i, tup, rd, ...) case i: asm volatile(rd : "=v"(t[0]), "=v"(t[1]), "=v"(t[2]), "=v"(t[3]), "=v"(t[4]), "=v"(t[5]), \
+    "=v"(t[6]), "=v"(t[7]), "=v"(t[8]), "=v"(t[9]), "=v"(t[10]), "=v"(t[11]), "=v"(t[12]), "=v"(t[13]), "=v"(t[14]), "=v"(t[15])); break;
+  switch (ac) { USP_U_ACC16(USP_MU_READ) }
+#undef USP_MU_READ
+#pragma unroll
+  for (int r = 0; r < 16; ++r) o[r] = t[r];
+#endif
+}
+USP_DEV void acc_settle() { asm volatile("s_nop 15\n\ts_nop 3" ::: "memory"); }
+
+template <int... I, class F> USP_DEV void static_for_seq(std::integer_sequence<int, I...>, F&& f) { (f(std::integral_constant<int, I>{}), ...); }
+template <int N, class F> USP_DEV void static_for(F&& f) { static_for_seq(std::make_integer_sequence<int, N>{}, f); }
+
+USP_DEV void pin_vgpr4(u32x4& x) {
+#if defined(__HIP_DEVICE_COMPILE__)
+  asm volatile("" : "+v"(x));
+#endif
+}
+USP_DEV void load_resident16_v(u32x4 (&f0)[8], u32x4 (&f1)[8], const char* r0, const char* r1) {
+#if defined(__HIP_DEVICE_COMPILE__)
+  asm volatile("global_load_dwordx4 %0, %16, off\n\tglobal_load_dwordx4 %1, %16, off offset:32\n\t"
+               "global_load_dwordx4 %2, %16, off offset:64\n\tglobal_load_dwordx4 %3, %16, off offset:96\n\t"
+               "global_load_dwordx4 %4, %16, off offset:128\n\tglobal_load_dwordx4 %5, %16, off offset:160\n\t"
+               "global_load_dwordx4 %6, %16, off offset:192\n\tglobal_load_dwordx4 %7, %16, off offset:224\n\t"
+               "global_load_dwordx4 %8, %17, off\n\tglobal_load_dwordx4 %9, %17, off offset:32\n\t"
+               "global_load_dwordx4 %10, %17, off offset:64\n\tglobal_load_dwordx4 %11, %17, off offset:96\n\t"
+               "global_load_dwordx4 %12, %17, off offset:128\n\tglobal_load_dwordx4 %13, %17, off offset:160\n\t"
+               "global_load_dwordx4 %14, %17, off offset:192\n\tglobal_load_dwordx4 %15, %17, off offset:224\n\t"
+               "s_waitcnt vmcnt(0)"
+               : "=&v"(f0[0]), "=&v"(f0[1]), "=&v"(f0[2]), "=&v"(f0[3]), "=&v"(f0[4]), "=&v"(f0[5]), "=&v"(f0[6]), "=&v"(f0[7]),
+                 "=&v"(f1[0]), "=&v"(f1[1]), "=&v"(f1[2]), "=&v"(f1[3]), "=&v"(f1[4]), "=&v"(f1[5]), "=&v"(f1[6]), "=&v"(f1[7])
+               : "v"(r0), "v"(r1) : "memory");
+#endif
+}
+
+template <int DT, bool CAUSAL>
+__global__ __launch_bounds__(256, 1) void flash_bwd_dkdv64u_kernel(const BwdParams ) {
+  using E = Elem<DT>;
+  using U = MU<DT>;
+  constexpr int D = 128, OWN = 256;
+  constexpr int ROWB = D * 2;
+  constexpr int TILEB = kTile * ROWB;
+  constexpr int STATB = 2 * kTile * 4;
+  constexpr int BUFB = 2 * TILEB + STATB;
+  constexpr int NBUF = 3;
+  constexpr int NKT = D / 16, NDJ = D / 32;
+
+  extern __shared__ __attribute__((aligned(16))) char smem_raw[];
+  USP_LDS char* smem = lds_block_at_zero(smem_raw);
+
+  const int tid = threadIdx.x;
+  const int lane = tid & 63;
+  const int wave = __builtin_amdgcn_readfirstlane(tid >> 6);
+  const int l31 = lane & 31;
+  const int hi = lane >> 5;
+  typedef const __attribute__((address_space(4))) BwdParams* KArgs;
+  KArgs p = (KArgs)__builtin_amdgcn_kernarg_segment_ptr();
+  asm volatile("" : "+s"(p));
+
+  const int dma_row = lane >> 4;
+  const int dma_c8 = ((lane & 15) ^ ((lane >> 4) << 2)) * 16;
+  const int q_voff = dma_row * (int)p->q_ss * 2 + dma_c8, do_voff = dma_row * (int)p->do_ss * 2 + dma_c8;
+  const int rd_base = l31 * ROWB + ((hi ^ tile_swz<D>(l31)) * 16);
+  const int tr_base = tr_read_offset<D>(lane & 15, (lane >> 4) & 1, hi, 0, 0);
+
+  const ItemWalk walk(p->n_items);
+  for (int pass = 0;; ++pass) {
+  int w = walk.at(pass);
+  if (w < 0) break;
+  asm volatile("" : "+s"(p));
+  w = walk.dealt(w, p->nblk);
+  const int blk = w % p->nblk;
+  int rest = w / p->nblk;
+  int g = 0, cut = 0;
+  if (p->qsplit > 1) { cut = rest % p->qsplit; rest /= p->qsplit; }
+  if (p->ngrp > 1) { g = rest % p->ngrp; rest /= p->ngrp; }
+  const int hkv = rest % p->Hkv, b = rest / p->Hkv;
+  const int gsub = p->gsub;
+  const int h0 = hkv * p->G + g * gsub;
+  const int own0 = blk * OWN;
+  const int off = p->causal_off;
+  const int ow = own0 + wave * 64;
+
+  u32x4 kf[2][NKT], vf[2][NKT];
+  {
+    const char *pk[2], *pv[2];
+#pragma unroll
+    for (int kb = 0; kb < 2; ++kb) {
+      const int orow = ow + 32 * kb + l31;
+      const int orow_c = orow < p->Sk ? orow : p->Sk - 1;
+      pk[kb] = p->k + 2 * (b * p->k_sb + (int64_t)orow_c * p->k_ss + hkv * p->k_sh) + 16 * hi;
+      pv[kb] = p->v + 2 * (b * p->v_sb + (int64_t)orow_c * p->v_ss + hkv * p->v_sh) + 16 * hi;
+    }
+    load_resident16_v(kf[0], kf[1], pk[0], pk[1]);
+    load_resident16_v(vf[0], vf[1], pv[0], pv[1]);
+  }
+  const float c2 = p->scale_log2;
+  const float neg_inv_scale = -__builtin_amdgcn_rcpf(p->scale);
+
+  int t_end = (p->Sq + kTile - 1) / kTile;
+  int t_begin = usp_first_row_tile(own0, CAUSAL, off, t_end, kTile);
+  if (p->qsplit > 1) {
+    const int per = usp_run_length(t_begin, t_end, p->qsplit);
+    t_begin = usp_run_begin(t_begin, t_end, per, cut);
+    t_end = usp_run_end(t_begin, t_end, per);
+  }
+  const int n_iter = t_end - t_begin;
+
+  const int64_t tb1 = (int64_t)kTile * p->q_ss * 2, tb2 = (int64_t)kTile * p->do_ss * 2;
+  int q_step = 4 * (int)p->q_ss * 2 - 1024, do_step = 4 * (int)p->do_ss * 2 - 1024;
+  const int q_rowb = (int)p->q_ss * 2, do_rowb = (int)p->do_ss * 2;
+  int lds_q = wave * 4096, lds_d = TILEB + wave * 4096;
+  const char *q_cur = nullptr, *do_cur = nullptr;
+  int rows_g = 0;
+
+  const float *lse_h = nullptr, *dl_h = nullptr;
+  int st_row = 0;
+  float st_lse = 0.f, st_delta = 0.f;
+  bool st_in = false;
+  const bool stat_wave = wave == 0;
+  auto pf_head = [&](int h) {
+    q_cur = p->q + 2 * (b * p->q_sb + h * p->q_sh) + t_begin * tb1 + (int64_t)wave * 16 * q_rowb;
+    do_cur = p->dout + 2 * (b * p->do_sb + h * p->do_sh) + t_begin * tb2 + (int64_t)wave * 16 * do_rowb;
+    rows_g = p->Sq - t_begin * kTile - 16 * wave;
+    lse_h = p->lse + b * p->lse_sb + h * p->lse_sh;
+    dl_h = p->delta + b * p->dl_sb + h * p->dl_sh;
+    st_row = t_begin * kTile;
+  };
+  u32x4 q_rs, do_rs;
+  int dma_buf = 0;
+  auto dma_open = [&](int buf) {
+    q_rs = make_rsrc_rows(q_cur, rows_g, 16, q_rowb, 2 * D);
+    do_rs = make_rsrc_rows(do_cur, rows_g, 16, do_rowb, 2 * D);
+    dma_buf = buf;
+    q_cur += tb1;
+    do_cur += tb2;
+    rows_g -= kTile;
+  };
+  auto stats_fetch = [&]() {
+    if (stat_wave) {
+      const int r = st_row + lane;
+      st_in = r < p->Sq;
+      const int rc = st_in ? r : p->Sq - 1;
+      const float* pl = lse_h + rc;
+      const float* pd = dl_h + rc;
+      asm volatile("global_load_dword %0, %2, off\n\tglobal_load_dword %1, %3, off" : "=&v"(st_lse), "=&v"(st_delta) : "v"(pl), "v"(pd) : "memory");
+    }
+    st_row += kTile;
+  };
+  auto dma_piece = [&](int n) {
+    asm volatile("" : "+s"(lds_q), "+s"(lds_d), "+s"(q_step), "+s"(do_step));
+    const int i = n & 3;
+    if (n < 4) lds_dma16_asm(q_rs, lds_q + dma_buf * BUFB, q_voff ^ (16 * i), i * q_step, i);
+    else lds_dma16_asm(do_rs, lds_d + dma_buf * BUFB, do_voff ^ (16 * i), i * do_step, i);
+  };
+  auto stats_store = [&](int buf) {
+    if (stat_wave) {
+      asm volatile("" : "+v"(st_lse), "+v"(st_delta));
+      const float l2 = (st_in && st_lse != USP_NEG_INF) ? st_lse * neg_inv_scale : -__builtin_inff();
+      *(USP_LDS float*)(smem + buf * BUFB + 2 * TILEB + 4 * lane) = l2;
+      *(USP_LDS float*)(smem + buf * BUFB + 2 * TILEB + 4 * kTile + 4 * lane) = st_in ? -st_delta : 0.f;
+    }
+  };
+
+  u32x4 zfrag = u32x4{0u, 0u, 0u, 0u};
+  asm volatile("" : "+v"(zfrag));
+#pragma unroll
+  for (int kb = 0; kb < 2; ++kb)
+#pragma unroll
+    for (int dj = 0; dj < NDJ; ++dj) { U::zero(4 * kb + dj, zfrag); U::zero(8 + 4 * kb + dj, zfrag); }
+
+  const int n_mask = usp_masked_row_tiles(ow, CAUSAL, off, t_begin, n_iter, kTile);
+  int tile_cur = t_begin, buf_a = 0;
+USP_TM(
+  uint64_t tm_body = 0, tm_drain = 0, tm_bar = 0, tm_last = __builtin_amdgcn_s_memtime();
+)
+  auto step = [&](auto mask_c) __attribute__((always_inline)) {
+    constexpr bool MASK = decltype(mask_c)::value;
+    constexpr int PE0 = kU_PE0, PE1 = kU_PE1, SE0 = kU_SE0, SE1 = kU_SE1, LA = kU_LA;
+    static_assert(PE0 >= 17 && PE1 <= 40 && PE1 > PE0 && (PE0 + (PE1 - PE0 + 1) / 2) <= 31, "P of k-step 0 in front of dV");
+    static_assert(SE0 >= 33 && SE1 <= 55 && SE1 > SE0 && (SE0 + (SE1 - SE0 + 1) / 2) <= 47, "dS of k-step 0 in front of dK");
+    static_assert(LA >= 1 && LA <= 7, "");
+    const int buf_n = buf_a + 1 == NBUF ? 0 : buf_a + 1;
+    stats_fetch();
+#pragma unroll
+    for (int kb = 0; kb < 2; ++kb)
+#pragma unroll
+      for (int t = 0; t < NKT; ++t) { pin_vgpr4(kf[kb][t]); pin_vgpr4(vf[kb][t]); }
+    const int s0 = tile_cur * kTile;
+    USP_LDS const char* stat = smem + buf_a * BUFB + 2 * TILEB + 16 * hi;
+    int kr = rd_base + buf_a * BUFB, tr = tr_base + buf_a * BUFB;
+    f32x16 sc[2], dp[2];
+    u32x4 pkp[2][2], pks[2][2];
+    u32x4 fr[2][32];
+    auto rd = [&](int h, int gf) {
+      const int j = gf & 7;
+      if (gf < 16) {
+        if (j == 0) asm volatile("" : "+v"(kr));
+        fr[h][gf] = *(USP_LDS const u32x4*)(smem + (kr ^ (32 * j)) + (gf < 8 ? 0 : TILEB) + h * 32 * ROWB);
+      } else {
+        if (j == 0) asm volatile("" : "+v"(tr));
+        const int k2 = j / NDJ, dj = j % NDJ;
+        USP_LDS const char* xb = smem + (gf < 24 ? TILEB : 0) + (2 * h + k2) * 16 * ROWB;
+        const u32x2 a0 = lds_read_tr16(xb + (tr ^ (64 * dj)));
+        const u32x2 a1 = lds_read_tr16(xb + (tr ^ (64 * dj + 32)) + 2048);
+        fr[h][gf] = u32x4{a0[0], a0[1], a1[0], a1[1]};
+      }
+    };
+    auto rd_stats = [&](int h, int which, int n) {
+      const int kb = n >> 2, j = n & 3;
+      const f32x4 t = *(USP_LDS const f32x4*)(stat + 4 * kTile * which + 128 * h + 32 * j);
+#pragma unroll
+      for (int e = 0; e < 4; ++e) (which ? dp : sc)[kb][4 * j + e] = t[e];
+    };
+    auto p_elem = [&](int n) {
+      const int k2 = n >> 4, kb = (n >> 3) & 1, r = 8 * k2 + (n & 7);
+      sc[kb][r] = fast_exp2(sc[kb][r] * c2);
+    };
+    auto p_pack = [&](int n) {
+      const int k2 = n >> 4, kb = (n >> 3) & 1, r = 8 * k2 + (n & 7);
+      if (r & 1) pkp[kb][k2][(r & 7) >> 1] = E::pack2(sc[kb][r - 1], sc[kb][r]);
+    };
+    auto s_elem = [&](int n) {
+      const int k2 = n >> 4, kb = (n >> 3) & 1, r = 8 * k2 + (n & 7);
+      const uint32_t wd = pkp[kb][k2][(r & 7) >> 1];
+      dp[kb][r] = ((r & 1) ? E::hi(wd) : E::lo(wd)) * dp[kb][r];
+      if (r & 1) pks[kb][k2][(r & 7) >> 1] = E::pack2(dp[kb][r - 1], dp[kb][r]);
+    };
+    constexpr int LAG = 2;
+    auto elem_slot = [&](int sl) {
+      if (sl >= PE0 && sl < PE1) {
+#pragma unroll
+        for (int n = (sl - PE0) * 32 / (PE1 - PE0); n < (sl - PE0 + 1) * 32 / (PE1 - PE0); ++n) {
+          p_elem(n);
+          if (n >= LAG) p_pack(n - LAG);
+        }
+        if (sl == PE1 - 1) {
+#pragma unroll
+          for (int n = 32 - LAG; n < 32; ++n) p_pack(n);
+        }
+      }
+      if (sl >= SE0 && sl < SE1) {
+#pragma unroll
+        for (int n = (sl - SE0) * 32 / (SE1 - SE0); n < (sl - SE0 + 1) * 32 / (SE1 - SE0); ++n) s_elem(n);
+      }
+    };
+    auto apply_mask = [&](int h) {
+#pragma unroll
+      for (int kb = 0; kb < 2; ++kb) {
+        const int d = ow + 32 * kb + l31 - off - s0 - 4 * hi - 32 * h;
+#pragma unroll
+        for (int r = 0; r < 16; ++r)
+          if (d > (r & 3) + 8 * (r >> 2)) sc[kb][r] = USP_NEG_INF;
+      }
+    };
+#pragma unroll
+    for (int gf = 0; gf < LA; ++gf) rd(0, gf);
+#pragma unroll
+    for (int n = 0; n < 8; ++n) rd_stats(0, 0, n);
+    __builtin_amdgcn_sched_barrier(0);
+    static_for<2>([&](auto h_c) __attribute__((always_inline)) {
+      constexpr int h = decltype(h_c)::value;
+      static_for<64>([&](auto sl_c) __attribute__((always_inline)) {
+        constexpr int sl = decltype(sl_c)::value;
+        constexpr int gf = sl >> 1, kb = sl & 1, j = gf & 7;
+        if (gf < 8) {
+          U::template chain<MASK || j == 0>(sc[kb], fr[h][gf], kf[kb][j]);
+        } else if (gf < 16) {
+          U::template chain<MASK || j == 0>(dp[kb], fr[h][gf], vf[kb][j]);
+        } else if (gf < 24) {
+          U::template grad<MASK>(4 * kb + j % NDJ, fr[h][gf], pkp[kb][j / NDJ]);
+        } else {
+          U::template grad<MASK>(8 + 4 * kb + j % NDJ, fr[h][gf], pks[kb][j / NDJ]);
+        }
+        if (h == 0 && sl == 0) {
+          __builtin_amdgcn_sched_barrier(0);
+          dma_open(buf_n);
+        }
+        if (kb == 0) {
+          if (gf + LA < 32) rd(h, gf + LA);
+          else if (h == 0) rd(1, gf + LA - 32);
+        }
+        if (sl >= 6 && sl < 14) rd_stats(h, 1, sl - 6);
+        if (h == 0 && sl >= 54 && sl < 62) rd_stats(1, 0, sl - 54);
+        if (h == 0 && sl >= 1 && sl <= 8) dma_piece(sl - 1);
+        elem_slot(sl);
+        __builtin_amdgcn_sched_barrier(0);
+        if (MASK && sl == 15) {
+          mfma_settle(sc);
+          apply_mask(h);
+          __builtin_amdgcn_sched_barrier(0);
+        }
+      });
+    });
+    buf_a = buf_n;
+    ++tile_cur;
+    USP_TM(const uint64_t tm0 = __builtin_amdgcn_s_memtime();)
+    dma_drain();
+    USP_TM(const uint64_t tm1 = __builtin_amdgcn_s_memtime();)
+    stats_store(buf_n);
+    __syncthreads();
+    USP_TM(const uint64_t tm2 = __builtin_amdgcn_s_memtime();
+           tm_body += tm0 - tm_last; tm_drain += tm1 - tm0; tm_bar += tm2 - tm1; tm_last = tm2;)
+  };
+  const std::integral_constant<bool, false> plain;
+  const std::integral_constant<bool, true> masked;
+  auto open_head = [&](int h) {
+    pf_head(h);
+    stats_fetch();
+    dma_open(0);
+#pragma unroll
+    for (int n = 0; n < 8; ++n) dma_piece(n);
+    dma_drain();
+    stats_store(0);
+    __syncthreads();
+    tile_cur = t_begin; buf_a = 0;
+  };
+  for (int hh = 0; hh < gsub; ++hh) {
+    open_head(h0 + hh);
+    int it = 0;
+    __builtin_amdgcn_s_waitcnt(0x0f70);
+    for (; it < n_mask; ++it) step(masked);
+    __builtin_amdgcn_s_waitcnt(0x0f70);
+    for (; it < n_iter; ++it) step(plain);
+  }
+
+  acc_settle();
+  asm volatile("" : "+s"(p));
+#pragma unroll
+  for (int ten = 0; ten < 2; ++ten) {
+    const bool wide = !p->split && (p->wide16 & (ten == 0 ? 4 : 2)) != 0;
+    const float mul = ten == 0 ? 1.f : p->scale;
+#pragma unroll
+    for (int kb = 0; kb < 2; ++kb) {
+      const int orow = ow + 32 * kb + l31;
+      f32x16 acc[NDJ];
+#pragma unroll
+      for (int dj = 0; dj < NDJ; ++dj) acc_read(8 * ten + 4 * kb + dj, acc[dj]);
+      if (wide) {
+        const int orow_c = orow < p->Sk ? orow : 0;
+        char* row16 = ten == 0 ? p->dv16 + 2 * (b * p->dv16_sb + (int64_t)orow_c * p->dv16_ss + hkv * p->dv16_sh)
+                               : p->dk16 + 2 * (b * p->dk16_sb + (int64_t)orow_c * p->dk16_ss + hkv * p->dk16_sh);
+        store_row16_wide<E, NDJ>(row16, acc, mul, hi, orow < p->Sk);
+      } else if (orow < p->Sk) {
+        float* o32;
+        char* o16 = nullptr;
+        int accf;
+        if (p->split) {
+          const int64_t wo = (((int64_t)(g * p->qsplit + cut) * p->ws_rows + (int64_t)b * p->Sk + orow) * p->Hkv + hkv) * D;
+          o32 = (ten == 0 ? p->ws_dv : p->ws_dk) + wo; accf = 0;
+        } else if (ten == 0) {
+          o32 = p->dv + b * p->dv_sb + (int64_t)orow * p->dv_ss + hkv * p->dv_sh; accf = p->accum_dv;
+          if (p->dv16) o16 = p->dv16 + 2 * (b * p->dv16_sb + (int64_t)orow * p->dv16_ss + hkv * p->dv16_sh);
+        } else {
+          o32 = p->dk + b * p->dk_sb + (int64_t)orow * p->dk_ss + hkv * p->dk_sh; accf = p->accum_dk;
+          if (p->dk16) o16 = p->dk16 + 2 * (b * p->dk16_sb + (int64_t)orow * p->dk16_ss + hkv * p->dk16_sh);
+        }
+        store_row32_acc<E, NDJ>(o32, o16, acc, mul, hi, accf);
+      }
+    }
+  }
+USP_TM(
+  if (pass == 0 && lane == 0 && (blockIdx.x % 61) == 0)
+    printf("TM wg %3d wave %d blk %2d n_iter %3d n_mask %d : body %8llu drain %7llu barrier %7llu  (per tile %5llu / %4llu / %4llu)\n",
+           (int)blockIdx.x, wave, blk, n_iter, n_mask, (unsigned long long)tm_body, (unsigned long long)tm_drain,
+           (unsigned long long)tm_bar, (unsigned long long)(tm_body / (n_iter * gsub + 1)), (unsigned long long)(tm_drain / (n_iter * gsub + 1)),
+           (unsigned long long)(tm_bar / (n_iter * gsub + 1)));
+)
+  }
+}
+
+bool dkdv64u_serves(const BwdParams& p_in) { return dkdv64_serves(p_in); }
+
+bool launch_dkdv64u(const BwdParams& p_in, int dtype, bool causal, hipStream_t st, int* rc) {
+  if (!dkdv64u_serves(p_in)) return false;
+  BwdParams p = p_in;
+  p.wide16 = ((p.dk16 && !p.accum_dk && tensor_aligned(p.dk16, p.dk16_sb, p.dk16_ss, p.dk16_sh, 16, 8)) ? 2 : 0) |
+             ((p.dv16 && !p.accum_dv && tensor_aligned(p.dv16, p.dv16_sb, p.dv16_ss, p.dv16_sh, 16, 8)) ? 4 : 0);
+  p.nblk = (p.Sk + 255) / 256;
+  p.n_items = p.B * p.Hkv * p.nblk * p.ngrp * p.qsplit;
+  const int grid = persistent_grid(p.n_items, device_cus(), p.interleave);
+  constexpr size_t lds = 3 * (2 * kTile * 128 * 2 + 2 * kTile * 4);
+  with_dtype_causal(dtype, causal, [&](auto dt, auto c) {
+    hipLaunchKernelGGL((flash_bwd_dkdv64u_kernel<decltype(dt)::value, decltype(c)::value>), dim3(grid), dim3(256), lds, st, p);
+  });
+  *rc = launched();
+  return true;
+}
+
+}
```

After: 1052, median of 6. 2.0% higher.
